# Meng-333/FastDiffSR

Hardware: AMD Instinct MI355X
Metric: 256x256 SR images/sec at T=20 (higher is better)
Workload: dtype f16x3; 1 GPU; x4 64->256, batch=16/GPU, T=20, random-init FastDiffSR UNet (inner 64, mults 1-2-4-4), 256x256, conv arithmetic f16x3 (BASELINE configs[1]); batch_per_gpu=16, global_batch=16, noise=drawn in the loop by the engine (Philox4x32-10), hipgraph=False, parallelism=dp1 (independent batches, weights broadcast once)

## Files before the change

### fastdiffsr_amd/csrc/fdsr_act_io.h

```cpp
#pragma once
#include "fdsr_kernels.h"

namespace fdsr {

typedef float f32x4 __attribute__((ext_vector_type(4)));
typedef float f32x16 __attribute__((ext_vector_type(16)));

__device__ __forceinline__ float bf16_bits_to_f32(unsigned v) { return __builtin_bit_cast(float, v << 16); }
__device__ __forceinline__ unsigned short f32_to_bf16_bits(float v) { return __builtin_bit_cast(unsigned short, (__bf16)v); }
__device__ __forceinline__ void sat_check(int* flag, f32x4 v, float lim) {
  const float m = fmaxf(fmaxf(fabsf(v.x), fabsf(v.y)), fmaxf(fabsf(v.z), fabsf(v.w)));
  if (m > lim) *flag = 1;
}
__device__ __forceinline__ int xcc_id() {
  unsigned v;
  asm volatile("s_getreg_b32 %0, hwreg(HW_REG_XCC_ID)" : "=s"(v));
  return (int)(v & (GSUM_SHARDS - 1));
}
__device__ __forceinline__ void gsum_add(unsigned long long* tab, int n, int npairs, int pair, int shard, float s1, float s2) {
  unsigned long long* g = tab + (((size_t)n * GSUM_SHARDS + shard) * npairs + pair) * 2;
  const long long a = __float2ll_rn(s1 * (float)(1 << GSUM_BITS1)), b = __float2ll_rn(s2 * (float)(1 << GSUM_BITS2));
  __hip_atomic_fetch_add(g, (unsigned long long)a, __ATOMIC_RELAXED, __HIP_MEMORY_SCOPE_WORKGROUP);
  __hip_atomic_fetch_add(g + 1, (unsigned long long)b, __ATOMIC_RELAXED, __HIP_MEMORY_SCOPE_WORKGROUP);
}
__device__ __forceinline__ float f16_bits_to_f32(unsigned v) { return (float)__builtin_bit_cast(_Float16, (unsigned short)v); }
__device__ __forceinline__ unsigned short f32_to_f16_bits(float v) {
  return __builtin_bit_cast(unsigned short, (_Float16)__builtin_amdgcn_fmed3f(v, -65504.0f, 65504.0f));
}
template <int PREC> struct ActIO;
template <> struct ActIO<PREC_F16X3> {
  typedef f32x4 Quad;
  static constexpr int ESZ = 4;
  static __device__ __forceinline__ Quad load4(const float* base, size_t idx) { return *reinterpret_cast<const f32x4*>(base + idx); }
  static __device__ __forceinline__ f32x4 widen(Quad q) { return q; }
  static __device__ __forceinline__ float load1(const float* base, size_t idx) { return base[idx]; }
  static __device__ __forceinline__ void store1(float* base, size_t idx, float v) { base[idx] = v; }
};
template <> struct ActIO<PREC_BF16> {
  typedef uint2 Quad;
  static constexpr int ESZ = 2;
  static __device__ __forceinline__ Quad load4(const float* base, size_t idx) {
    return *reinterpret_cast<const uint2*>(reinterpret_cast<const unsigned short*>(base) + idx);
  }
  static __device__ __forceinline__ f32x4 widen(Quad q) {
    f32x4 r = {__builtin_bit_cast(float, q.x << 16), __builtin_bit_cast(float, q.x & 0xffff0000u),
               __builtin_bit_cast(float, q.y << 16), __builtin_bit_cast(float, q.y & 0xffff0000u)};
    return r;
  }
  static __device__ __forceinline__ float load1(const float* base, size_t idx) {
    return bf16_bits_to_f32(reinterpret_cast<const unsigned short*>(base)[idx]);
  }
  static __device__ __forceinline__ void store1(float* base, size_t idx, float v) {
    reinterpret_cast<unsigned short*>(base)[idx] = f32_to_bf16_bits(v);
  }
};
template <> struct ActIO<PREC_F16> {
  typedef uint2 Quad;
  static constexpr int ESZ = 2;
  static __device__ __forceinline__ Quad load4(const float* base, size_t idx) {
    return *reinterpret_cast<const uint2*>(reinterpret_cast<const unsigned short*>(base) + idx);
  }
  static __device__ __forceinline__ f32x4 widen(Quad q) {
    typedef _Float16 h2 __attribute__((ext_vector_type(2)));
    const h2 a = __builtin_bit_cast(h2, q.x), b = __builtin_bit_cast(h2, q.y);
    f32x4 r = {(float)a[0], (float)a[1], (float)b[0], (float)b[1]};
    return r;
  }
  static __device__ __forceinline__ float load1(const float* base, size_t idx) {
    return f16_bits_to_f32(reinterpret_cast<const unsigned short*>(base)[idx]);
  }
  static __device__ __forceinline__ void store1(float* base, size_t idx, float v) {
    reinterpret_cast<unsigned short*>(base)[idx] = f32_to_f16_bits(v);
  }
};

template <int PREC>
__device__ __forceinline__ uint2 pack4_16(f32x4 v) {
  uint2 pk;
  if (PREC == PREC_F16) {
    pk.x = (unsigned)f32_to_f16_bits(v[0]) | ((unsigned)f32_to_f16_bits(v[1]) << 16);
    pk.y = (unsigned)f32_to_f16_bits(v[2]) | ((unsigned)f32_to_f16_bits(v[3]) << 16);
  } else {
    pk.x = (unsigned)f32_to_bf16_bits(v[0]) | ((unsigned)f32_to_bf16_bits(v[1]) << 16);
    pk.y = (unsigned)f32_to_bf16_bits(v[2]) | ((unsigned)f32_to_bf16_bits(v[3]) << 16);
  }
  return pk;
}
__device__ __forceinline__ unsigned short f32_to_16_bits(float v, int code) { return code == 2 ? f32_to_f16_bits(v) : f32_to_bf16_bits(v); }
template <int PREC>
__device__ __forceinline__ uint2 stage4_16(f32x4 v) {
  if (PREC == PREC_F16) {
    typedef _Float16 h4 __attribute__((ext_vector_type(4)));
    const h4 hb = {(_Float16)v[0], (_Float16)v[1], (_Float16)v[2], (_Float16)v[3]};
    return __builtin_bit_cast(uint2, hb);
  }
  typedef __bf16 b4_ __attribute__((ext_vector_type(4)));
  const b4_ hb = {(__bf16)v[0], (__bf16)v[1], (__bf16)v[2], (__bf16)v[3]};
  return __builtin_bit_cast(uint2, hb);
}
template <int PREC>
__device__ __forceinline__ f32x4 mfma16_k32(uint4 a, uint4 b, f32x4 c) {
  typedef __bf16 b8_ __attribute__((ext_vector_type(8)));
  typedef _Float16 h8_ __attribute__((ext_vector_type(8)));
  if (PREC == PREC_BF16) return __builtin_amdgcn_mfma_f32_16x16x32_bf16(__builtin_bit_cast(b8_, a), __builtin_bit_cast(b8_, b), c, 0, 0, 0);
  return __builtin_amdgcn_mfma_f32_16x16x32_f16(__builtin_bit_cast(h8_, a), __builtin_bit_cast(h8_, b), c, 0, 0, 0);
}
template <int PREC>
__device__ __forceinline__ f32x16 mfma32_k16(uint4 a, uint4 b, f32x16 c) {
  typedef __bf16 b8_ __attribute__((ext_vector_type(8)));
  typedef _Float16 h8_ __attribute__((ext_vector_type(8)));
  if (PREC == PREC_BF16) return __builtin_amdgcn_mfma_f32_32x32x16_bf16(__builtin_bit_cast(b8_, a), __builtin_bit_cast(b8_, b), c, 0, 0, 0);
  return __builtin_amdgcn_mfma_f32_32x32x16_f16(__builtin_bit_cast(h8_, a), __builtin_bit_cast(h8_, b), c, 0, 0, 0);
}

}
```

### fastdiffsr_amd/csrc/fdsr_conv_dev.h

```cpp
#pragma once
#include "fdsr_kernels.h"
#include "fdsr_act_io.h"

namespace fdsr {

typedef _Float16 h8 __attribute__((ext_vector_type(8)));
typedef _Float16 h4 __attribute__((ext_vector_type(4)));
typedef _Float16 h2 __attribute__((ext_vector_type(2)));
typedef __bf16 b8 __attribute__((ext_vector_type(8)));
typedef __bf16 b4 __attribute__((ext_vector_type(4)));
typedef unsigned u32x4 __attribute__((ext_vector_type(4)));

__device__ __forceinline__ float silu_fast(float v) { return v * __builtin_amdgcn_rcpf(1.0f + __expf(-v)); }

__device__ __forceinline__ int xcd_block_id(int b, int nwg) {
  const int q8 = nwg >> 3, r8 = nwg & 7, xcd = b & 7, k = b >> 3;
  return (xcd < r8 ? xcd * (q8 + 1) : r8 * (q8 + 1) + (xcd - r8) * q8) + k;
}

__device__ __forceinline__ void split2_mix(float a, float b, float lim, unsigned& hi, unsigned& lo) {
  const float ca = __builtin_amdgcn_fmed3f(a, -lim, lim), cb = __builtin_amdgcn_fmed3f(b, -lim, lim);
  const h2 h = {(_Float16)ca, (_Float16)cb};
  hi = __builtin_bit_cast(unsigned, h);
  asm("v_fma_mixlo_f16 %0, %1, -1.0, %2 op_sel:[0,0,0] op_sel_hi:[1,0,0]" : "=v"(lo) : "v"(hi), "v"(ca));
  asm("v_fma_mixhi_f16 %0, %1, -1.0, %2 op_sel:[1,0,0] op_sel_hi:[1,0,0]" : "+v"(lo) : "v"(hi), "v"(cb));
}
__device__ __forceinline__ void split4_mix(f32x4 v, float lim, uint2& hi, uint2& lo) {
#pragma unroll
  for (int e = 0; e < 4; ++e) v[e] = __builtin_amdgcn_fmed3f(v[e], -lim, lim);
  {
    const h2 h0 = {(_Float16)v[0], (_Float16)v[1]}, h1 = {(_Float16)v[2], (_Float16)v[3]};
    hi.x = __builtin_bit_cast(unsigned, h0);
    hi.y = __builtin_bit_cast(unsigned, h1);
  }
  asm("v_fma_mixlo_f16 %0, %1, -1.0, %2 op_sel:[0,0,0] op_sel_hi:[1,0,0]" : "=v"(lo.x) : "v"(hi.x), "v"(v[0]));
  asm("v_fma_mixhi_f16 %0, %1, -1.0, %2 op_sel:[1,0,0] op_sel_hi:[1,0,0]" : "+v"(lo.x) : "v"(hi.x), "v"(v[1]));
  asm("v_fma_mixlo_f16 %0, %1, -1.0, %2 op_sel:[0,0,0] op_sel_hi:[1,0,0]" : "=v"(lo.y) : "v"(hi.y), "v"(v[2]));
  asm("v_fma_mixhi_f16 %0, %1, -1.0, %2 op_sel:[1,0,0] op_sel_hi:[1,0,0]" : "+v"(lo.y) : "v"(hi.y), "v"(v[3]));
}
__device__ __forceinline__ void split4_2step(f32x4 v, float lim, h4& hi, h4& lo) {
#pragma unroll
  for (int e = 0; e < 4; ++e) v[e] = __builtin_amdgcn_fmed3f(v[e], -lim, lim);
  hi = h4{(_Float16)v.x, (_Float16)v.y, (_Float16)v.z, (_Float16)v.w};
  lo = h4{(_Float16)(v.x - (float)hi.x), (_Float16)(v.y - (float)hi.y), (_Float16)(v.z - (float)hi.z), (_Float16)(v.w - (float)hi.w)};
}

struct ChunkSrc {
  const float* base;
  int Cs, cc;
  int cbase;
  bool gn;
};
template <bool RIDER>
__device__ __forceinline__ ChunkSrc chunk_src(const ConvParams& p, int kc, int KC, int nk, int q, bool gn) {
  ChunkSrc s;
  s.cbase = kc * KC;
  s.gn = gn;
  if (RIDER && kc >= nk) {
    s.cbase -= nk * KC;
    s.gn = false;
    if (s.cbase < p.Cr0) { s.base = p.xr0; s.Cs = p.Cr0; s.cc = s.cbase + q * 4; }
    else { s.base = p.xr1; s.Cs = p.Cr1; s.cc = s.cbase - p.Cr0 + q * 4; }
  } else if (s.cbase < p.C0) { s.base = p.x0; s.Cs = p.C0; s.cc = s.cbase + q * 4; }
  else { s.base = p.x1; s.Cs = p.C1; s.cc = s.cbase - p.C0 + q * 4; }
  return s;
}

__device__ __forceinline__ f32x4 gn_act4(f32x4 v, f32x4 sc, f32x4 sh, bool plain) {
  v = v * sc + sh;
  if (!plain) { v.x = silu_fast(v.x); v.y = silu_fast(v.y); v.z = silu_fast(v.z); v.w = silu_fast(v.w); }
  return v;
}
__device__ __forceinline__ f32x4 drop4(f32x4 v, unsigned mask_bytes, float scale) {
#pragma unroll
  for (int e = 0; e < 4; ++e) v[e] *= (float)((mask_bytes >> (8 * e)) & 0xffu) * scale;
  return v;
}

template <bool RIDER>
__device__ __forceinline__ float epi_add1(const float* bias, const float* bias_r, const float* tembp, float tmul, int c) {
  float a = bias[c];
  if (RIDER) a += bias_r[c];
  a += tmul * tembp[c];
  return a;
}
template <bool RIDER>
__device__ __forceinline__ f32x4 epi_add4(const float* bias, const float* bias_r, const float* tembp, float tmul, int c) {
  f32x4 a;
#pragma unroll
  for (int r = 0; r < 4; ++r) a[r] = epi_add1<RIDER>(bias, bias_r, tembp, tmul, c + r);
  return a;
}
template <int PREC, bool OUT16>
__device__ __forceinline__ void put4(float* out, size_t idx, f32x4 v) {
  if (OUT16) *reinterpret_cast<uint2*>(reinterpret_cast<unsigned short*>(out) + idx) = pack4_16<PREC>(v);
  else *reinterpret_cast<f32x4*>(out + idx) = v;
}


}
```

### fastdiffsr_amd/csrc/fdsr_conv_h.hip

```cpp
#include "fdsr_conv_dev.h"

#include <algorithm>
#include <cstdlib>
#include <type_traits>

namespace fdsr {

template <int KS, int STRIDE, bool UP, int TH, int WN, int PREC, int KSUB>
struct ConvHCfg {
  static constexpr int TW = 32, NW = 8;
  static constexpr int KC = 16 * KSUB;
  static constexpr int NP = PREC == PREC_F16X3 ? 2 : 1;
  static constexpr int WNP = PREC == PREC_BF16 ? 1 : 2;
  static constexpr int ROWB = NP * 32 * KSUB + 16;
  static constexpr int PAD = KS / 2;
  static constexpr int HH = (TH - 1) * STRIDE + KS;
  static constexpr int HWD = (TW - 1) * STRIDE + KS;
  static constexpr int NPIX = HH * HWD;
  static constexpr int WM = NW / WN;
  static constexpr int BN = 32 * WN;
  static constexpr int MB = TH / WM;
  static constexpr int NT = 64 * NW;
  static constexpr int Q4 = 4 * KSUB;
  static constexpr int RPP = NT / Q4;
  static constexpr int NIN = (NPIX + RPP - 1) / RPP;
  static constexpr int T = KS * KS * KSUB;
  static_assert(KSUB == 1 || KS == 1, "sub-chunking is for 1x1 only");
  static constexpr int BUF_BYTES = (NPIX * ROWB + 15) / 16 * 16;
  static_assert(TH % WM == 0, "TH must be a multiple of WM");
};

#ifdef CONVH_STAMPS
__device__ unsigned long long g_h_stamps[256][2][64];
#define H_STAMP()                                                                                                  \
  do {                                                                                                             \
    if (stamp_on && si < 64) g_h_stamps[blockIdx.x][wave == 0 ? 0 : 1][si] = __builtin_amdgcn_s_memtime();         \
    ++si;                                                                                                          \
  } while (0)
#else
#define H_STAMP() do {} while (0)
#endif

template <int KS, int STRIDE, bool UP, int TH, int WN, int PREC, int KSUB, bool RIDER = false>
__global__ void __launch_bounds__(512, 2) conv_mfma_h_kernel(const ConvParams p) {
  static_assert(!RIDER || (KS == 3 && STRIDE == 1 && !UP && KSUB == 1), "the rider rides the stride-1 3x3 kernels");
  using Cfg = ConvHCfg<KS, STRIDE, UP, TH, WN, PREC, KSUB>;
  constexpr int TW = Cfg::TW, KC = Cfg::KC, NP = Cfg::NP, ROWB = Cfg::ROWB, PAD = Cfg::PAD, HWD = Cfg::HWD;
  constexpr int NPIX = Cfg::NPIX, WM = Cfg::WM, BN = Cfg::BN, MB = Cfg::MB, RPP = Cfg::RPP, NIN = Cfg::NIN, T = Cfg::T, Q4 = Cfg::Q4, NW = Cfg::NW;

  extern __shared__ __attribute__((aligned(16))) unsigned char smem_h[];
  unsigned char* sBuf0 = smem_h;
  unsigned char* sBuf1 = smem_h + Cfg::BUF_BYTES;
  const int Cin = p.C0 + p.C1;

  const int tid = threadIdx.x, lane = tid & 63, wave = tid >> 6;
  const int wn = wave % WN, wm = wave / WN;

  const int nco = p.Cout_pad / BN;
  const int tilesX = (p.Wout + TW - 1) / TW, tilesY = (p.Hout + TH - 1) / TH;
  int bid = xcd_block_id(blockIdx.x, gridDim.x);
  const int SK = p.ksplit > 1 ? p.ksplit : 1;
  const int ksi = bid % SK;
  bid /= SK;
  const int cot = bid % nco;
  int pt = bid / nco;
  const int tx = pt % tilesX;
  pt /= tilesX;
  const int ty = pt % tilesY;
  const int n = pt / tilesY;
  const int oy0 = ty * TH, ox0 = tx * TW, co0 = cot * BN;

  const bool gn = p.gn_scale != nullptr;
#ifdef CONVH_STAMPS
  int si = 0;
  const bool stamp_on = KS == 3 && STRIDE == 1 && !UP && !RIDER && PREC == CONVH_STAMP_PREC && lane == 0 && (wave == 0 || wave == 7) &&
                        blockIdx.x < 256 && Cin == CONVH_STAMP_CIN && p.Cout == CONVH_STAMP_COUT;
#endif
  H_STAMP();

  const int q = tid % Q4, row0 = tid / Q4;
  int in_pix[NIN];
#pragma unroll
  for (int i = 0; i < NIN; ++i) {
    const int pix = row0 + i * RPP;
    int v = -2;
    if (pix < NPIX) {
      const int hy = pix / HWD, hx = pix % HWD;
      const int iy = oy0 * STRIDE - PAD + hy, ix = ox0 * STRIDE - PAD + hx;
      if (UP) {
        const bool ok = iy >= 0 && iy < p.Hout && ix >= 0 && ix < p.Wout;
        v = ok ? (n * p.Hin + (iy >> 1)) * p.Win + (ix >> 1) : -1;
      } else {
        const bool ok = iy >= 0 && iy < p.Hin && ix >= 0 && ix < p.Win;
        v = ok ? (n * p.Hin + iy) * p.Win + ix : -1;
      }
    }
    in_pix[i] = v;
  }

  using IO = ActIO<PREC>;
  typedef typename IO::Quad Quad;
  Quad rin[NIN];
  Quad rin2[RIDER ? NIN : 1];
  f32x4 rsc = {1.f, 1.f, 1.f, 1.f}, rsh = {0.f, 0.f, 0.f, 0.f};
  const int nk = p.Cin_pad / KC;
  auto prefetch_to = [&](int kc, Quad* rin) {
    const ChunkSrc src = chunk_src<RIDER>(p, kc, KC, nk, q, gn);
    if (src.gn) {
      rsc = *reinterpret_cast<const f32x4*>(p.gn_scale + (size_t)n * Cin + src.cbase + q * 4);
      rsh = *reinterpret_cast<const f32x4*>(p.gn_shift + (size_t)n * Cin + src.cbase + q * 4);
    }
#pragma unroll
    for (int i = 0; i < NIN; ++i)
      rin[i] = IO::load4(src.base, (size_t)(in_pix[i] < 0 ? 0 : in_pix[i]) * src.Cs + src.cc);
  };
  auto prefetch = [&](int kc) { prefetch_to(kc, rin); };
  auto stage_from = [&](int kc, unsigned char* buf, const Quad* rin) {
    const f32x4 sc = rsc, sh = rsh;
#pragma unroll
    for (int i = 0; i < NIN; ++i) {
      if (NIN * RPP > NPIX && i == NIN - 1 && row0 + i * RPP >= NPIX) continue;
      f32x4 v = IO::widen(rin[i]);
      if (gn && !(RIDER && kc >= nk)) {
        v = gn_act4(v, sc, sh, p.gn_plain);
      } else if (PREC == PREC_F16X3 && p.sat_flag) {
        sat_check(p.sat_flag, v, 65504.f);
      }
      const float keep = in_pix[i] >= 0 ? 1.f : 0.f;
      const float lim = in_pix[i] >= 0 ? 65504.f : 0.f;
      unsigned char* dst = buf + (row0 + i * RPP) * ROWB + (q >> 2) * (NP * 32) + (q & 3) * 8;
      if (PREC == PREC_F16X3) {
        h4 hi, lo;
        split4_2step(v, lim, hi, lo);
        *reinterpret_cast<h4*>(dst) = hi;
        *reinterpret_cast<h4*>(dst + 32) = lo;
      } else {
        v = v * keep;
        *reinterpret_cast<uint2*>(dst) = stage4_16<PREC>(v);
      }
    }
  };
  auto stage = [&](int kc, unsigned char* buf) { stage_from(kc, buf, rin); };

  const uint4* wq = reinterpret_cast<const uint4*>(p.wq);
  const int nkt = RIDER ? nk + p.nkr : nk;
  uint4 Bf[T][NP];
  auto load_b_tap = [&](int kc, int tap) {
    const int ts = tap / KSUB, sub = tap % KSUB;
    const uint4* src = wq + ((((size_t)cot * (nk * KSUB) + kc * KSUB + sub) * WN + wn) * (KS * KS) + ts) * (Cfg::WNP * 64) + lane;
    if (RIDER && kc >= nk)
      src = reinterpret_cast<const uint4*>(p.wq_r) + (((size_t)cot * p.nkr + (kc - nk)) * WN + wn) * (Cfg::WNP * 64) + lane;
#pragma unroll
    for (int pl = 0; pl < NP; ++pl) Bf[tap][pl] = src[pl * 64];
  };

  const int r31 = lane & 31, h = lane >> 5;
  int abase[MB];
#pragma unroll
  for (int mb = 0; mb < MB; ++mb) {
    const int br = wm + mb * WM;
    abase[mb] = ((br * STRIDE) * HWD + r31 * STRIDE) * ROWB + 16 * h;
  }

  f32x16 acc[MB];
#pragma unroll
  for (int mb = 0; mb < MB; ++mb)
#pragma unroll
    for (int i = 0; i < 16; ++i) acc[mb][i] = 0.f;

  const int kc0 = ksi * nkt / SK, kc1 = (ksi + 1) * nkt / SK;
#pragma unroll
  for (int tap = 0; tap < T; ++tap)
    if (tap == 0 || !(RIDER && kc0 >= nk)) load_b_tap(kc0, tap);
  prefetch(kc0);
  H_STAMP();
  stage(kc0, sBuf0);
  H_STAMP();
  if (kc0 + 1 < kc1) prefetch(kc0 + 1);
  __syncthreads();
  H_STAMP();

  uint4 Af[2][MB][NP];
  const unsigned char* arow[MB];
  auto load_a = [&](int slot, int tap) {
    const int ts = tap / KSUB, sub = tap % KSUB;
    const int ky = ts / KS, kx = ts % KS;
    const int aoff = (ky * HWD + kx) * ROWB + sub * (NP * 32);
#pragma unroll
    for (int mb = 0; mb < MB; ++mb)
#pragma unroll
      for (int pl = 0; pl < NP; ++pl)
        Af[slot][mb][pl] = *reinterpret_cast<const uint4*>(arow[mb] + aoff + 32 * pl);
  };

  const int kcm = RIDER ? (kc1 < nk ? kc1 : nk) : kc1;
  for (int kc = kc0; kc < kcm; ++kc) {
    unsigned char* cur = ((kc - kc0) & 1) ? sBuf1 : sBuf0;
    unsigned char* nxt = ((kc - kc0) & 1) ? sBuf0 : sBuf1;
    const bool more = kc + 1 < kc1;
    const bool next_rider = RIDER && kc + 1 >= nk;
#pragma unroll
    for (int mb = 0; mb < MB; ++mb) arow[mb] = cur + abase[mb];
    load_a(0, 0);
#pragma unroll
    for (int tap = 0; tap < T; ++tap) {
      if (tap + 1 < T) load_a((tap + 1) & 1, tap + 1);
#pragma unroll
      for (int mb = 0; mb < MB; ++mb) {
        const uint4 ahi = Af[tap & 1][mb][0];
        if (PREC == PREC_F16X3) {
          const uint4 alo = Af[tap & 1][mb][NP - 1];
          acc[mb] = __builtin_amdgcn_mfma_f32_32x32x16_f16(__builtin_bit_cast(h8, alo), __builtin_bit_cast(h8, Bf[tap][0]), acc[mb], 0, 0, 0);
          acc[mb] = __builtin_amdgcn_mfma_f32_32x32x16_f16(__builtin_bit_cast(h8, ahi), __builtin_bit_cast(h8, Bf[tap][NP - 1]), acc[mb], 0, 0, 0);
          acc[mb] = __builtin_amdgcn_mfma_f32_32x32x16_f16(__builtin_bit_cast(h8, ahi), __builtin_bit_cast(h8, Bf[tap][0]), acc[mb], 0, 0, 0);
        } else {
          acc[mb] = mfma32_k16<PREC>(ahi, Bf[tap][0], acc[mb]);
        }
      }
      if (more && (tap == 0 || !next_rider)) load_b_tap(kc + 1, tap);
      if (tap == T / 2 && more) {
        H_STAMP();
#ifdef CONVH_KO_STAGE
        if (PREC != CONVH_KO_STAGE) {
          stage(kc + 1, nxt);
          if (kc + 2 < kc1) prefetch(kc + 2);
        }
#else
        stage(kc + 1, nxt);
        if (kc + 2 < kc1) prefetch(kc + 2);
#endif
        H_STAMP();
      }
    }
    H_STAMP();
    __syncthreads();
    H_STAMP();
  }
  if (RIDER && kc1 > nk) {
    if (kc0 < nk) {
      const float ratio = (p.w_inv_scale_dev ? *p.w_inv_scale_dev : p.w_inv_scale) / (p.w_inv_scale_r_dev ? *p.w_inv_scale_r_dev : p.w_inv_scale_r);
#pragma unroll
      for (int mb = 0; mb < MB; ++mb) acc[mb] *= ratio;
    }
    const int k0 = kc0 > nk ? kc0 : nk;
    if (k0 + 2 < kc1) prefetch_to(k0 + 2, rin2);
    auto rider_chunk = [&](int kc, Quad* r1, Quad* r2) {
      unsigned char* cur = ((kc - kc0) & 1) ? sBuf1 : sBuf0;
      unsigned char* nxt = ((kc - kc0) & 1) ? sBuf0 : sBuf1;
      (void)r2;
#pragma unroll
      for (int mb = 0; mb < MB; ++mb) arow[mb] = cur + abase[mb];
      load_a(0, T / 2);
#pragma unroll
      for (int mb = 0; mb < MB; ++mb) {
        const uint4 ahi = Af[0][mb][0];
        if (PREC == PREC_F16X3) {
          const uint4 alo = Af[0][mb][NP - 1];
          acc[mb] = __builtin_amdgcn_mfma_f32_32x32x16_f16(__builtin_bit_cast(h8, alo), __builtin_bit_cast(h8, Bf[0][0]), acc[mb], 0, 0, 0);
          acc[mb] = __builtin_amdgcn_mfma_f32_32x32x16_f16(__builtin_bit_cast(h8, ahi), __builtin_bit_cast(h8, Bf[0][NP - 1]), acc[mb], 0, 0, 0);
          acc[mb] = __builtin_amdgcn_mfma_f32_32x32x16_f16(__builtin_bit_cast(h8, ahi), __builtin_bit_cast(h8, Bf[0][0]), acc[mb], 0, 0, 0);
        } else {
          acc[mb] = mfma32_k16<PREC>(ahi, Bf[0][0], acc[mb]);
        }
      }
      if (kc + 1 < kc1) {
        load_b_tap(kc + 1, 0);
        stage_from(kc + 1, nxt, r1);
        if (kc + 3 < kc1) prefetch_to(kc + 3, r1);
      }
      __syncthreads();
    };
    for (int kc = k0; kc < kc1; kc += 2) {
      rider_chunk(kc, rin, rin2);
      if (kc + 1 < kc1) rider_chunk(kc + 1, rin2, rin);
    }
  }

  const int co = co0 + wn * 32 + r31;
  const bool cok = co < p.Cout;
  const float* tembp = p.temb ? p.temb + (size_t)n * p.temb_stride + p.temb_off : p.bias;
  const float add = epi_add1<RIDER>(p.bias, p.bias_r, tembp, p.temb ? 1.f : 0.f, cok ? co : 0);
  float s1 = 0.f, s2 = 0.f;
  const float winv_m = p.w_inv_scale_dev ? *p.w_inv_scale_dev : p.w_inv_scale;
  const float winv = RIDER ? (p.w_inv_scale_r_dev ? *p.w_inv_scale_r_dev : p.w_inv_scale_r) : winv_m;
  if (RIDER && kc1 <= nk) {
    const float ratio = winv_m / winv;
#pragma unroll
    for (int mb = 0; mb < MB; ++mb) acc[mb] *= ratio;
  }
  const bool interior = (oy0 + TH <= p.Hout) && (ox0 + TW <= p.Wout) && (co0 + BN <= p.Cout);
  if (SK > 1) {
    float* sb = p.kscratch + (size_t)ksi * p.N * p.Hout * p.Wout * p.Cout;
    if (interior) {
      float* obase = sb + ((size_t)(n * p.Hout + oy0 + wm) * p.Wout + ox0 + 4 * h) * p.Cout + co;
      const size_t rstride = (size_t)WM * p.Wout * p.Cout;
#pragma unroll
      for (int mb = 0; mb < MB; ++mb)
#pragma unroll
        for (int i = 0; i < 16; ++i) obase[mb * rstride + (size_t)((i & 3) + 8 * (i >> 2)) * p.Cout] = acc[mb][i];
    } else {
#pragma unroll
      for (int mb = 0; mb < MB; ++mb)
#pragma unroll
        for (int i = 0; i < 16; ++i) {
          const int oy = oy0 + wm + mb * WM, ox = ox0 + (i & 3) + 8 * (i >> 2) + 4 * h;
          if (cok && oy < p.Hout && ox < p.Wout) sb[((size_t)(n * p.Hout + oy) * p.Wout + ox) * p.Cout + co] = acc[mb][i];
        }
    }
    return;
  }
  auto epilogue = [&](auto out16_tag) {
    constexpr bool OUT16 = decltype(out16_tag)::value;
    auto put = [&](size_t idx, float v) {
      if (OUT16) reinterpret_cast<unsigned short*>(p.out)[idx] = PREC == PREC_F16 ? f32_to_f16_bits(v) : f32_to_bf16_bits(v);
      else p.out[idx] = v;
    };
    if (interior) {
      const size_t obase = ((size_t)(n * p.Hout + oy0 + wm) * p.Wout + ox0 + 4 * h) * p.Cout + co;
      const size_t rstride = (size_t)WM * p.Wout * p.Cout;
      float rv[MB][16];
      if (p.res) {
#pragma unroll
        for (int mb = 0; mb < MB; ++mb)
#pragma unroll
          for (int i = 0; i < 16; ++i) rv[mb][i] = IO::load1(p.res, obase + mb * rstride + (size_t)((i & 3) + 8 * (i >> 2)) * p.Cout);
      } else {
#pragma unroll
        for (int mb = 0; mb < MB; ++mb)
#pragma unroll
          for (int i = 0; i < 16; ++i) rv[mb][i] = 0.f;
      }
#pragma unroll
      for (int mb = 0; mb < MB; ++mb)
#pragma unroll
        for (int i = 0; i < 16; ++i) {
          const float v = acc[mb][i] * winv + add + rv[mb][i];
          put(obase + mb * rstride + (size_t)((i & 3) + 8 * (i >> 2)) * p.Cout, v);
          s1 += v;
          s2 += v * v;
        }
    } else {
      float rv[MB][16];
      if (p.res) {
#pragma unroll
        for (int mb = 0; mb < MB; ++mb)
#pragma unroll
          for (int i = 0; i < 16; ++i) {
            const int oy = oy0 + wm + mb * WM, ox = ox0 + (i & 3) + 8 * (i >> 2) + 4 * h;
            const bool ok = cok && oy < p.Hout && ox < p.Wout;
            rv[mb][i] = ok ? IO::load1(p.res, ((size_t)(n * p.Hout + oy) * p.Wout + ox) * p.Cout + co) : 0.f;
          }
      }
#pragma unroll
      for (int mb = 0; mb < MB; ++mb)
#pragma unroll
        for (int i = 0; i < 16; ++i) {
          const int oy = oy0 + wm + mb * WM, ox = ox0 + (i & 3) + 8 * (i >> 2) + 4 * h;
          if (cok && oy < p.Hout && ox < p.Wout) {
            float v = acc[mb][i] * winv + add;
            if (p.res) v += rv[mb][i];
            put(((size_t)(n * p.Hout + oy) * p.Wout + ox) * p.Cout + co, v);
            s1 += v;
            s2 += v * v;
          }
        }
    }
  };
  H_STAMP();
  if (prec_is16(PREC) && !p.out_f32) epilogue(std::true_type{});
  else epilogue(std::false_type{});
  H_STAMP();
  if (p.part_out) {
    float* sp = reinterpret_cast<float*>(smem_h);
    s1 += __shfl_xor(s1, 32, 64);
    s2 += __shfl_xor(s2, 32, 64);
    if (h == 0) {
      sp[(wm * BN + wn * 32 + r31) * 2 + 0] = s1;
      sp[(wm * BN + wn * 32 + r31) * 2 + 1] = s2;
    }
    __syncthreads();
    if (tid < BN && co0 + tid < p.Cout) {
      float a = 0.f, b = 0.f;
#pragma unroll
      for (int w = 0; w < WM; ++w) { a += sp[(w * BN + tid) * 2 + 0]; b += sp[(w * BN + tid) * 2 + 1]; }
      float* dst = p.part_out + (((size_t)n * (tilesX * tilesY) + ty * tilesX + tx) * p.Cout + co0 + tid) * 2;
      dst[0] = a;
      dst[1] = b;
    }
  }
  H_STAMP();
}

#ifdef CONVH_STAMPS
extern "C" int fdsr_diag_convh_stamps(unsigned long long* dst, size_t count) {
  return (int)hipMemcpyFromSymbol(dst, HIP_SYMBOL(g_h_stamps), count * sizeof(unsigned long long), 0, hipMemcpyDeviceToHost);
}
#endif

template <int NS, bool OUT16, bool CB32>
__global__ void __launch_bounds__(256) splitk_reduce_kernel(const ConvParams p, const int cb) {
  __shared__ float sred[256 * 8];
  const int tilesX = (p.Wout + 31) / 32;
  const int tile = blockIdx.x, n = blockIdx.y;
  const int tx = tile % tilesX, ty = tile / tilesX;
  const int cq = CB32 ? 8 : cb >> 2, groups = CB32 ? 32 : 256 / cq, cbase = blockIdx.z * cb;
  const int tid = threadIdx.x, c4 = tid % cq, g = tid / cq;
  const int cch = cbase + c4 * 4;
  const bool has_r = p.xr0 != nullptr, has_t = p.temb != nullptr, has_res = p.res != nullptr;
  const f32x4 bias = *reinterpret_cast<const f32x4*>(p.bias + cch);
  const f32x4 bias_r = *reinterpret_cast<const f32x4*>(has_r ? p.bias_r + cch : p.bias + cbase);
  const f32x4 temb = *reinterpret_cast<const f32x4*>(has_t ? p.temb + (size_t)n * p.temb_stride + p.temb_off + cch : p.bias + cbase);
  const float* wdev = has_r ? p.w_inv_scale_r_dev : p.w_inv_scale_dev;
  const float wload = *(wdev ? wdev : p.bias);
  const size_t slice = (size_t)p.N * p.Hout * p.Wout * p.Cout;
  const int last = p.ksplit - 1;
  const float* resp = has_res ? p.res : p.out;
  constexpr int NPX = CB32 ? 2 : 1;
  f32x4 s1 = {0.f, 0.f, 0.f, 0.f}, s2 = {0.f, 0.f, 0.f, 0.f};
  auto pixels = [&](int px0) __attribute__((always_inline)) {
    f32x4 sl[NPX][NS], rv[NPX];
    size_t o[NPX];
    bool ok[NPX];
#pragma unroll
    for (int i = 0; i < NPX; ++i) {
      const int px = px0 + i * groups;
      const int oy = ty * 2 + (px >> 5), ox = tx * 32 + (px & 31);
      ok[i] = g < groups && px < 64 && oy < p.Hout && ox < p.Wout;
      o[i] = ((size_t)(n * p.Hout + min(oy, p.Hout - 1)) * p.Wout + min(ox, p.Wout - 1)) * p.Cout + cch;
#pragma unroll
      for (int s = 0; s < NS; ++s) sl[i][s] = *reinterpret_cast<const f32x4*>(p.kscratch + (size_t)min(s, last) * slice + o[i]);
      if (OUT16) rv[i] = p.out_bf16 == 2 ? ActIO<PREC_F16>::widen(ActIO<PREC_F16>::load4(resp, o[i])) : ActIO<PREC_BF16>::widen(ActIO<PREC_BF16>::load4(resp, o[i]));
      else rv[i] = *reinterpret_cast<const f32x4*>(resp + o[i]);
    }
    __builtin_amdgcn_sched_barrier(0);
    const float winv = wdev ? wload : (has_r ? p.w_inv_scale_r : p.w_inv_scale);
    f32x4 add = bias;
#pragma unroll
    for (int e = 0; e < 4; ++e) {
      add[e] += has_r ? bias_r[e] : 0.f;
      add[e] += has_t ? temb[e] : 0.f;
    }
#pragma unroll
    for (int i = 0; i < NPX; ++i) {
      f32x4 a = sl[i][0];
#pragma unroll
      for (int s = 1; s < NS; ++s)
#pragma unroll
        for (int e = 0; e < 4; ++e) a[e] += s <= last ? sl[i][s][e] : 0.f;
      a = a * winv + add;
#pragma unroll
      for (int e = 0; e < 4; ++e) a[e] += has_res ? rv[i][e] : 0.f;
#pragma unroll
      for (int e = 0; e < 4; ++e) {
        const float v = ok[i] ? a[e] : 0.f;
        s1[e] += v;
        s2[e] += v * v;
      }
      if (ok[i]) {
        if (OUT16) {
          *reinterpret_cast<uint2*>(reinterpret_cast<unsigned short*>(p.out) + o[i]) = p.out_bf16 == 2 ? pack4_16<PREC_F16>(a) : pack4_16<PREC_BF16>(a);
        } else {
          *reinterpret_cast<f32x4*>(p.out + o[i]) = a;
        }
      }
    }
  };
  if (CB32) pixels(g);
  else for (int px0 = g; px0 < 64; px0 += groups) pixels(px0);
  if (p.part_out) {
    if (g < groups) {
      *reinterpret_cast<f32x4*>(sred + (g * cq + c4) * 8) = s1;
      *reinterpret_cast<f32x4*>(sred + (g * cq + c4) * 8 + 4) = s2;
    }
    __syncthreads();
    if (tid < cq) {
      f32x4 a = {0.f, 0.f, 0.f, 0.f}, b = a;
      for (int gg = 0; gg < groups; ++gg) {
        a += *reinterpret_cast<const f32x4*>(sred + (gg * cq + tid) * 8);
        b += *reinterpret_cast<const f32x4*>(sred + (gg * cq + tid) * 8 + 4);
      }
      float* dst = p.part_out + (((size_t)n * gridDim.x + tile) * p.Cout + cbase + tid * 4) * 2;
#pragma unroll
      for (int e = 0; e < 4; ++e) { dst[2 * e] = a[e]; dst[2 * e + 1] = b[e]; }
      if (p.gsum_out) {
        const int pair = (cbase + tid * 4) >> 1;
        const int xcd = xcc_id();
        gsum_add(p.gsum_out, n, p.Cout >> 1, pair, xcd, a[0] + a[1], b[0] + b[1]);
        gsum_add(p.gsum_out, n, p.Cout >> 1, pair + 1, xcd, a[2] + a[3], b[2] + b[3]);
      }
    }
  }
}

static hipError_t launch_splitk_reduce(const ConvParams& q, int rt, int cb, hipStream_t s) {
  const dim3 grid(rt, q.N, q.Cout / cb), block(256);
#define SKR(NS_)                                                                                                   \
  if (q.ksplit <= NS_) {                                                                                           \
    if (cb == 32) {                                                                                                \
      if (q.out_bf16) hipLaunchKernelGGL((splitk_reduce_kernel<NS_, true, true>), grid, block, 0, s, q, cb);       \
      else hipLaunchKernelGGL((splitk_reduce_kernel<NS_, false, true>), grid, block, 0, s, q, cb);                 \
    } else {                                                                                                       \
      if (q.out_bf16) hipLaunchKernelGGL((splitk_reduce_kernel<NS_, true, false>), grid, block, 0, s, q, cb);      \
      else hipLaunchKernelGGL((splitk_reduce_kernel<NS_, false, false>), grid, block, 0, s, q, cb);                \
    }                                                                                                              \
    return hipGetLastError();                                                                                      \
  }
  SKR(2) SKR(4) SKR(8) SKR(16)
#undef SKR
  return hipErrorInvalidValue;
}

template <int KS, int STRIDE, bool UP, int TH, int WN, int PREC, int KSUB, bool RIDER = false>
static hipError_t launch_h_t(const ConvParams& p, hipStream_t s, int* tiles) {
  using Cfg = ConvHCfg<KS, STRIDE, UP, TH, WN, PREC, KSUB>;
  auto kfn = conv_mfma_h_kernel<KS, STRIDE, UP, TH, WN, PREC, KSUB, RIDER>;
  const size_t lds = (size_t)2 * Cfg::BUF_BYTES;
  const int tilesX = (p.Wout + Cfg::TW - 1) / Cfg::TW, tilesY = (p.Hout + TH - 1) / TH;
  if (tiles) *tiles = tilesX * tilesY;
  const int sk = p.ksplit > 1 ? p.ksplit : 1;
  const int nwg = p.N * tilesX * tilesY * (p.Cout_pad / Cfg::BN) * sk;
  ConvParams q = p;
  q.out_bf16 = p.out_f32 ? 0 : prec_act16(PREC);
  if (KS == 3 && STRIDE == 1 && !UP && KSUB == 1 && (PREC == PREC_F16X3 || prec_is16(PREC)) && conv_k32_ok(TH, WN, PREC, q)) {
    const hipError_t e = launch_conv_k32(TH, WN, PREC, q, nwg, s);
    if (e != hipSuccess) return e;
  } else {
    if (p.gb_x0 || p.drop_mask || p.gs0) return hipErrorInvalidValue;
    hipLaunchKernelGGL(kfn, dim3(nwg), dim3(Cfg::NT), lds, s, q);
  }
  if (sk > 1 && (g_tun.knockout & 2)) {
    if (tiles) *tiles = ((p.Wout + 31) / 32) * ((p.Hout + 1) / 2);
  } else if (sk > 1) {
    const int rt = ((p.Wout + 31) / 32) * ((p.Hout + 1) / 2);
    if (tiles) *tiles = rt;
    const int cb = p.Cout % 32 == 0 ? 32 : p.Cout;
    const hipError_t e = launch_splitk_reduce(q, rt, cb, s);
    if (e != hipSuccess) return e;
  }
  return hipGetLastError();
}

template <int KS, int STRIDE, bool UP, int TH, int WN, int PREC, int KSUB, bool RIDER = false>
static hipError_t init_h_t() {
  auto kfn = conv_mfma_h_kernel<KS, STRIDE, UP, TH, WN, PREC, KSUB, RIDER>;
  return hipFuncSetAttribute(reinterpret_cast<const void*>(kfn), hipFuncAttributeMaxDynamicSharedMemorySize, 160 * 1024);
}

#define FDSR_CONVH_SHAPES(X)                                                                                   \
  X(3, 1, false, 8, 4, 1) X(3, 1, false, 4, 4, 1) X(3, 1, false, 16, 2, 1) X(3, 1, false, 8, 2, 1) X(3, 1, false, 4, 2, 1) \
  X(3, 1, false, 16, 1, 1) X(3, 1, false, 8, 1, 1) X(3, 1, false, 4, 8, 1) X(3, 1, false, 2, 8, 1)                       \
  X(3, 1, true, 4, 8, 1) X(3, 1, true, 2, 8, 1) X(3, 2, false, 4, 8, 1)                                                  \
  X(3, 1, true, 8, 4, 1) X(3, 1, true, 4, 4, 1) X(3, 1, true, 16, 2, 1) X(3, 1, true, 8, 2, 1) X(3, 1, true, 4, 2, 1)      \
  X(3, 2, false, 4, 4, 1) X(3, 2, false, 4, 2, 1)                                                                        \
  X(1, 1, false, 8, 4, 1) X(1, 1, false, 4, 4, 1) X(1, 1, false, 16, 2, 1) X(1, 1, false, 8, 2, 1) X(1, 1, false, 4, 2, 1) \
  X(1, 1, false, 16, 1, 1) X(1, 1, false, 8, 1, 1) X(1, 1, false, 4, 8, 1) X(1, 1, false, 2, 8, 1)                       \
  X(1, 1, false, 8, 4, 4) X(1, 1, false, 4, 4, 4) X(1, 1, false, 8, 2, 4) X(1, 1, false, 4, 2, 4)                         \
  X(1, 1, false, 8, 1, 4) X(1, 1, false, 4, 8, 4) X(1, 1, false, 2, 8, 4)

#define FDSR_CONVH_RIDER_SHAPES(XR) \
  XR(8, 4) XR(4, 4) XR(16, 2) XR(8, 2) XR(4, 2) XR(16, 1) XR(8, 1) XR(4, 8) XR(2, 8)

void conv_h_config(ConvKind kind, int Cout, int* TH, int* WN) {
  *WN = Cout >= 256 ? 8 : (Cout >= 128 ? 4 : (Cout >= 64 ? 2 : 1));
  if ((kind == CONV3_S2 || kind == CONV3_UP) && *WN == 1) *WN = 2;
  *TH = kind == CONV3_S2 ? 4 : 8;
}

static int pick_th(ConvKind kind, int WN, int ksub, const ConvParams& p) {
  if (kind == CONV3_S2) return 4;
  const int WM = 8 / WN;
  const int tilesX = (p.Wout + 31) / 32, nco = p.Cout_pad / (32 * WN);
  int best = -1;
  for (int th = 16; th >= 2; th >>= 1) {
    if (th % WM || th / WM > 4) continue;
    if (th < 4 && WN < 8) continue;
    if (ksub > 1 && th > 8) continue;
    const long wgs = (long)p.N * tilesX * ((p.Hout + th - 1) / th) * nco;
    best = th;
    if (wgs >= g_tun.th_min_wgs) break;
  }
  return best;
}

int conv_h_ksplit(ConvKind kind, int N, int Hout, int Wout, int Cout, int Cout_pad, int Cin_pad, int C0, int C1) {
  if (!g_tun.splitk || kind == CONV3_UP || (Cout & 3) || Cout > 1024) return 1;
  int TH, WN;
  conv_h_config(kind, Cout, &TH, &WN);
  const int ksub = (kind == CONV1 && Cin_pad % 64 == 0 && (C1 == 0 || C0 % 64 == 0)) ? 4 : 1;
  ConvParams p{};
  p.N = N; p.Hout = Hout; p.Wout = Wout; p.Cout_pad = Cout_pad;
  TH = pick_th(kind, WN, ksub, p);
  const long wgs = (long)N * ((Wout + 31) / 32) * ((Hout + TH - 1) / TH) * (Cout_pad / (32 * WN));
  const int nk = Cin_pad / (16 * ksub);
  const int target = g_tun.sk_target;
  if (wgs >= target) return 1;
  const int sk = (int)std::min<long>(std::min(16, nk / 2), (target + wgs - 1) / wgs);
  return sk >= 2 ? sk : 1;
}

bool conv_h_gnb_ok(ConvKind kind, int prec, const ConvParams& p) {
  if (kind != CONV3_S1 || prec != PREC_F16X3 || p.xr0 || p.res || p.ksplit > 1 || !p.out_f32 || p.gn_scale) return false;
  int TH, WN;
  conv_h_config(kind, p.Cout, &TH, &WN);
  if (WN == 2 && conv_k32_small_ok(kind, prec, p)) return true;
  TH = pick_th(kind, WN, 1, p);
  return conv_k32_ok(TH, WN, prec, p);
}

bool conv_h_drop_ok(ConvKind kind, int prec, const ConvParams& p) {
  if (kind != CONV3_S1 || !conv_k32_drop_ok(prec, p)) return false;
  int TH, WN;
  conv_h_config(kind, p.Cout, &TH, &WN);
  if (WN == 2 && conv_k32_small_ok(kind, prec, p)) return true;
  TH = pick_th(kind, WN, 1, p);
  return conv_k32_ok(TH, WN, prec, p);
}

bool conv_h_gnc_ok(ConvKind kind, int prec, const ConvParams& p) {
  if (!g_tun.gn_consumer || kind != CONV3_S1 || prec == PREC_F32) return false;
  int TH, WN;
  conv_h_config(kind, p.Cout, &TH, &WN);
  ConvParams q = p;
  q.gn_scale = q.gn_shift = reinterpret_cast<const float*>(p.gs_gamma);
  if ((WN == 2 || WN == 4) && conv_strip_ok(kind, prec, q)) return false;
  if (WN == 2 && conv_k32_small_ok(kind, prec, q)) return false;
  TH = pick_th(kind, WN, 1, p);
  return conv_k32_gnc_ok(TH, WN, prec, p);
}

bool conv_h_gsum_ok(ConvKind kind, int prec, const ConvParams& p, bool sub_pixel_up2) {
  if (!g_tun.gn_consumer || prec == PREC_F32 || (p.Cout & 3)) return false;
  if (p.ksplit > 1) return p.Cout % 32 == 0 && !(g_tun.knockout & 2);
  if (kind == CONV3_UP) return sub_pixel_up2 && conv_up2_k32_ok(prec, p);
  if (kind != CONV3_S1) return false;
  int TH, WN;
  conv_h_config(kind, p.Cout, &TH, &WN);
  if ((WN == 2 || WN == 4) && conv_strip_ok(kind, prec, p)) return false;
  if (WN == 2 && conv_k32_small_ok(kind, prec, p)) return true;
  TH = pick_th(kind, WN, 1, p);
  return conv_k32_ok(TH, WN, prec, p);
}

hipError_t launch_conv_h(ConvKind kind, int prec, const ConvParams& p, hipStream_t s, int* tiles) {
  int TH, WN;
  conv_h_config(kind, p.Cout, &TH, &WN);
  const int ksub = (kind == CONV1 && p.Cin_pad % 64 == 0 && (p.C1 == 0 || p.C0 % 64 == 0)) ? 4 : 1;
  if ((WN == 2 || WN == 4) && ksub == 1 && conv_strip_ok(kind, prec, p)) return launch_conv_strip(prec, p, WN, s, tiles);
  if (WN == 2 && ksub == 1 && conv_k32_small_ok(kind, prec, p)) return launch_conv_k32_small(prec, p, s, tiles);
  TH = pick_th(kind, WN, ksub, p);
  const int ks = kind == CONV1 ? 1 : 3, stride = kind == CONV3_S2 ? 2 : 1;
  const bool up = kind == CONV3_UP;
  if (p.xr0) {
    if (kind != CONV3_S1) return hipErrorInvalidValue;
#define XR(TH_, WN_)                                                                                     \
    if (TH == TH_ && WN == WN_)                                                                          \
      return prec == PREC_F16X3 ? launch_h_t<3, 1, false, TH_, WN_, PREC_F16X3, 1, true>(p, s, tiles)     \
                                : prec == PREC_F16 ? launch_h_t<3, 1, false, TH_, WN_, PREC_F16, 1, true>(p, s, tiles) : launch_h_t<3, 1, false, TH_, WN_, PREC_BF16, 1, true>(p, s, tiles);
    FDSR_CONVH_RIDER_SHAPES(XR)
#undef XR
    return hipErrorInvalidValue;
  }
#define X(KS_, ST_, UP_, TH_, WN_, KSUB_)                                                                \
  if (ks == KS_ && stride == ST_ && up == UP_ && TH == TH_ && WN == WN_ && ksub == KSUB_) {               \
    return prec == PREC_F16X3 ? launch_h_t<KS_, ST_, UP_, TH_, WN_, PREC_F16X3, KSUB_>(p, s, tiles)       \
                              : prec == PREC_F16 ? launch_h_t<KS_, ST_, UP_, TH_, WN_, PREC_F16, KSUB_>(p, s, tiles) : launch_h_t<KS_, ST_, UP_, TH_, WN_, PREC_BF16, KSUB_>(p, s, tiles);       \
  }
  FDSR_CONVH_SHAPES(X)
#undef X
  return hipErrorInvalidValue;
}

hipError_t kernels_h_init() {
  hipError_t e;
#define X(KS_, ST_, UP_, TH_, WN_, KSUB_)                                                          \
  if ((e = init_h_t<KS_, ST_, UP_, TH_, WN_, PREC_F16X3, KSUB_>()) != hipSuccess) return e;         \
  if ((e = init_h_t<KS_, ST_, UP_, TH_, WN_, PREC_BF16, KSUB_>()) != hipSuccess) return e; \
  if ((e = init_h_t<KS_, ST_, UP_, TH_, WN_, PREC_F16, KSUB_>()) != hipSuccess) return e;
  FDSR_CONVH_SHAPES(X)
#undef X
#define XR(TH_, WN_)                                                                                    \
  if ((e = init_h_t<3, 1, false, TH_, WN_, PREC_F16X3, 1, true>()) != hipSuccess) return e;              \
  if ((e = init_h_t<3, 1, false, TH_, WN_, PREC_BF16, 1, true>()) != hipSuccess) return e; \
  if ((e = init_h_t<3, 1, false, TH_, WN_, PREC_F16, 1, true>()) != hipSuccess) return e;
  FDSR_CONVH_RIDER_SHAPES(XR)
#undef XR
  if ((e = kernels_k32_init()) != hipSuccess) return e;
  return kernels_strip_init();
}

}
```

### fastdiffsr_amd/csrc/fdsr_conv_k32.hip

```cpp
#include "fdsr_conv_dev.h"

#include <type_traits>

namespace fdsr {

#ifndef XS_F16X3
#define XS_F16X3 2
#endif
#ifndef XS_BF16
#define XS_BF16 4
#endif
#ifndef K32_PIN
#define K32_PIN 1
#endif
#ifndef K32_RIDER2
#define K32_RIDER2 1
#endif
#ifndef K32_SPLIT
#define K32_SPLIT 1
#endif
#ifndef K32_SPLIT_BF16
#define K32_SPLIT_BF16 1
#endif
#ifndef K32_MIXSPLIT
#define K32_MIXSPLIT 1
#endif
#ifndef K32_PEEL
#define K32_PEEL 1
#endif
#ifndef K32_GNB_DIAG
#define K32_GNB_DIAG 0
#endif
#ifndef K32_DIAG
#define K32_DIAG 0
#endif
#ifndef K32_RFIRST
#define K32_RFIRST 1
#endif
#ifndef K32_PIN16
#define K32_PIN16 0
#endif

constexpr int K32_GNC_MAXC = 1024, K32_GNC_MAXP = K32_GNC_MAXC / 2 + 32, K32_GNC_LDS = K32_GNC_MAXP * 32 + K32_GNC_MAXC * 8;

template <int TH, int WN, int PREC, int NW_ = 8>
struct ConvK32Cfg {
  static constexpr int TW = 32, NW = NW_, KC = 32;
  static constexpr int NP = PREC == PREC_F16X3 ? 2 : 1;
  static constexpr int WNP = PREC == PREC_BF16 ? 1 : 2;
  static constexpr int ROWB = 64 * NP;
  static constexpr int HH = TH + 2, HWD = TW + 2, NPIX = HH * HWD;
  static constexpr int WM = NW / WN, BN = 32 * WN, MB = TH / WM;
  static constexpr int NT = 64 * NW;
  static constexpr int Q4 = KC / 4;
  static constexpr int RPP = NT / Q4;
  static constexpr int NIN = (NPIX + RPP - 1) / RPP;
  static constexpr int BUF_BYTES = NPIX * ROWB;
  static constexpr int LDS_BYTES = 2 * BUF_BYTES;
  static constexpr int R = 3;
  static constexpr int XS = PREC == PREC_F16X3 ? XS_F16X3 : (NW_ == 4 && TH == 8 ? 3 : XS_BF16);
  static_assert(MB == 4 || MB == 3 || MB == 2, "wave tile = 4 (small grids: 2; small workgroups in f16x3: 3) rows of 32 pixels");
  static_assert(((TH - WM + 2) * HWD + 16) * ROWB < 65536, "fragment offsets must fit the ds_read immediate");
};

template <int PREC>
__device__ __forceinline__ int k32_slot(int slot, int hx) {
  return PREC == PREC_F16X3 ? (slot ^ (hx & 7)) : (slot ^ ((hx >> 1) & 3));
}

template <int TH, int WN, int PREC, bool RIDER, int NW = 8, bool RF = (NW == 4), bool GNB = false, bool DROP = false, bool GNC = false>
__global__ void __launch_bounds__(64 * NW, 2) conv_k32_kernel(const ConvParams p) {
  using Cfg = ConvK32Cfg<TH, WN, PREC, NW>;
  constexpr int TW = Cfg::TW, KC = Cfg::KC, NP = Cfg::NP, ROWB = Cfg::ROWB, HWD = Cfg::HWD, NPIX = Cfg::NPIX;
  constexpr int WM = Cfg::WM, BN = Cfg::BN, MB = Cfg::MB, RPP = Cfg::RPP, NIN = Cfg::NIN, R = Cfg::R, XS = Cfg::XS;
  constexpr bool PIN = TH == 16 ? K32_PIN16 != 0 : K32_PIN != 0;
  constexpr bool CHAIN = PIN && !(RIDER && !RF);

  extern __shared__ __attribute__((aligned(16))) unsigned char smem_k[];
  unsigned char* sBuf0 = smem_k;
  unsigned char* sBuf1 = smem_k + Cfg::BUF_BYTES;
  const int Cin = p.C0 + p.C1;

  const int tid = threadIdx.x, lane = tid & 63, wave = tid >> 6;
  const int wn = wave % WN, wm = wave / WN;
  const int c15 = lane & 15, g = lane >> 4;

  const int nco = p.Cout_pad / BN;
  const int tilesX = (p.Wout + TW - 1) / TW, tilesY = (p.Hout + TH - 1) / TH;
  int bid = xcd_block_id(blockIdx.x, gridDim.x);
  const int SK = p.ksplit > 1 ? p.ksplit : 1;
  const int ksi = bid % SK;
  bid /= SK;
  const int cot = bid % nco;
  int pt = bid / nco;
  const int tx = pt % tilesX;
  pt /= tilesX;
  const int ty = pt % tilesY;
  const int n = pt / tilesY;
  const int oy0 = ty * TH, ox0 = tx * TW, co0 = cot * BN;

  const bool gn = GNC ? true : p.gn_scale != nullptr;

  if (NW == 4 && p.stagger > 0) {
    unsigned hwid;
    asm volatile("s_getreg_b32 %0, hwreg(HW_REG_HW_ID)" : "=s"(hwid));
    if ((hwid >> 16) & 1u) {
      const int n64 = p.stagger * (p.Cin_pad / KC + (RIDER ? p.nkr / 2 : 0));
      for (int i = 0; i < n64; i += 8) __builtin_amdgcn_s_sleep(8);
    }
  }

  const int q = tid & 7, row0 = tid >> 3;
  int in_pix[NIN];
  unsigned long long skeys = 0;
  static_assert(NIN <= 21, "swizzle keys are packed into one register pair");
#pragma unroll
  for (int i = 0; i < NIN; ++i) {
    const int pix = row0 + i * RPP;
    int v = -2;
    if (pix < NPIX) {
      const int hy = pix / HWD, hx = pix % HWD;
      const int iy = oy0 - 1 + hy, ix = ox0 - 1 + hx;
      const bool ok = iy >= 0 && iy < p.Hin && ix >= 0 && ix < p.Win;
      v = ok ? (n * p.Hin + iy) * p.Win + ix : -1;
      skeys |= (unsigned long long)k32_slot<PREC>(0, hx) << (3 * i);
    }
    in_pix[i] = v;
  }
  const int sbase = row0 * ROWB + 8 * (q & 1);

  using IO = ActIO<PREC>;
  typedef typename IO::Quad Quad;
  struct QM { Quad q; unsigned m; };
  constexpr bool RFIRST = RIDER && RF && K32_RFIRST != 0;
  constexpr bool SPLIT = K32_SPLIT != 0 && (PREC == PREC_F16X3 || K32_SPLIT_BF16 != 0) && (!RIDER || RFIRST);
  static_assert(!RFIRST || SPLIT, "the rider-first path writes whole chunks into rr1, which is sized for them only when SPLIT");
  constexpr int NA = SPLIT ? (NIN + 1) / 2 : NIN;
  typedef std::integral_constant<int, 0> I_0;
  typedef std::integral_constant<int, NA> I_A;
  typedef std::integral_constant<int, NIN> I_N;
  QM rin[NA];
  QM rr1[RIDER && SPLIT ? NIN : 1];
  QM rin2[RIDER && K32_RIDER2 && NW == 8 ? NIN : 1];
  f32x4 rsc = {1.f, 1.f, 1.f, 1.f}, rsh = {0.f, 0.f, 0.f, 0.f};
  const int nk = p.Cin_pad / KC;
  const int nk16 = p.Cin_pad / 16;
  const int nkr = RIDER ? p.nkr / 2 : 0;
  double* gnc_pr = reinterpret_cast<double*>(smem_k + Cfg::LDS_BYTES);
  float* gnc_sc = reinterpret_cast<float*>(smem_k + Cfg::LDS_BYTES + K32_GNC_MAXP * 32);
  float* gnc_sh = gnc_sc + K32_GNC_MAXC;
  int gnc_lo = 0, gnc_hi = 0, gnc_cpg = 1, gnc_q0 = 0, gnc_q1 = 0;
  constexpr int GNC_PT = (2 * K32_GNC_MAXP + Cfg::NT - 1) / Cfg::NT;
  uint4 gnc_ld[GNC ? GNC_PT : 1][GSUM_SHARDS / 2];
  constexpr int GNC_CT = (K32_GNC_MAXC + Cfg::NT - 1) / Cfg::NT;
  float gnc_gam[GNC ? GNC_CT : 1], gnc_bet[GNC ? GNC_CT : 1];
  auto gnc_issue = [&](int c_lo, int c_hi) __attribute__((always_inline)) {
    gnc_lo = c_lo; gnc_hi = c_hi;
    gnc_cpg = Cin / p.gs_G;
    gnc_q0 = (c_lo / gnc_cpg) * gnc_cpg / 2;
    gnc_q1 = ((c_hi - 1) / gnc_cpg + 1) * gnc_cpg / 2;
#pragma unroll
    for (int j = 0; j < GNC_PT; ++j) {
      const int u = tid + j * Cfg::NT, qc = min(gnc_q0 + (u >> 1), gnc_q1 - 1);
      const bool first = qc < (p.C0 >> 1);
      const unsigned long long* tab = first ? p.gs0 : p.gs1;
      const int np = (first ? p.C0 : p.C1) >> 1, ql = first ? qc : qc - (p.C0 >> 1);
#pragma unroll
      for (int sdx = 0; sdx < GSUM_SHARDS / 2; ++sdx)
        gnc_ld[j][sdx] = *reinterpret_cast<const uint4*>(tab + (((size_t)n * GSUM_SHARDS + (u & 1) * (GSUM_SHARDS / 2) + sdx) * np + ql) * 2);
    }
#pragma unroll
    for (int j = 0; j < GNC_CT; ++j) {
      const int cc = min(c_lo + tid + j * Cfg::NT, c_hi - 1);
      gnc_gam[j] = p.gs_gamma[cc];
      gnc_bet[j] = p.gs_beta[cc];
    }
  };
  auto gnc_finish = [&]() __attribute__((always_inline)) {
#pragma unroll
    for (int j = 0; j < GNC_PT; ++j) {
      const int u = tid + j * Cfg::NT, qi = gnc_q0 + (u >> 1);
      long long a = 0, b = 0;
#pragma unroll
      for (int sdx = 0; sdx < GSUM_SHARDS / 2; ++sdx) {
        a += (long long)(((unsigned long long)gnc_ld[j][sdx].y << 32) | gnc_ld[j][sdx].x);
        b += (long long)(((unsigned long long)gnc_ld[j][sdx].w << 32) | gnc_ld[j][sdx].z);
      }
      if (qi < gnc_q1) {
        gnc_pr[2 * u] = (double)a * (1.0 / (double)(1 << GSUM_BITS1));
        gnc_pr[2 * u + 1] = (double)b * (1.0 / (double)(1 << GSUM_BITS2));
      }
    }
    __syncthreads();
    const double inv = 1.0 / ((double)gnc_cpg * (double)p.Hin * (double)p.Win);
#pragma unroll
    for (int j = 0; j < GNC_CT; ++j) {
      const int c = gnc_lo + tid + j * Cfg::NT;
      if (c >= gnc_hi) break;
      const int g = c / gnc_cpg, hp = gnc_cpg >> 1;
      double s1 = 0.0, s2 = 0.0;
      for (int k = 0; k < 2 * hp; ++k) { s1 += gnc_pr[2 * (2 * (g * hp - gnc_q0) + k)]; s2 += gnc_pr[2 * (2 * (g * hp - gnc_q0) + k) + 1]; }
      const double mean = s1 * inv;
      double var = s2 * inv - mean * mean;
      var = var < 0.0 ? 0.0 : var;
      const double rstd = 1.0 / sqrt(var + (double)p.gs_eps);
      const float scv = (float)rstd * gnc_gam[j];
      gnc_sc[c - gnc_lo] = scv;
      gnc_sh[c - gnc_lo] = gnc_bet[j] - (float)mean * scv;
    }
    __syncthreads();
  };
  auto prefetch_rng = [&](int kc, QM* rin, auto i0_tag, auto i1_tag, bool load_gn) __attribute__((always_inline)) {
    constexpr int I0 = decltype(i0_tag)::value, I1 = decltype(i1_tag)::value;
    const ChunkSrc src = chunk_src<RIDER>(p, kc, KC, nk, q, gn);
    if (!GNC && src.gn && load_gn) {
      rsc = *reinterpret_cast<const f32x4*>(p.gn_scale + (size_t)n * Cin + src.cbase + q * 4);
      rsh = *reinterpret_cast<const f32x4*>(p.gn_shift + (size_t)n * Cin + src.cbase + q * 4);
    }
#pragma unroll
    for (int i = I0; i < I1; ++i) {
      const size_t pi = (size_t)(in_pix[i] < 0 ? 0 : in_pix[i]);
      rin[i - I0].q = IO::load4(src.base, pi * src.Cs + src.cc);
      if (DROP)
        rin[i - I0].m = *reinterpret_cast<const unsigned*>(p.drop_mask + ((RIDER && kc >= nk) ? (size_t)0 : pi * src.Cs + src.cc));
    }
  };
  auto prefetch_to = [&](int kc, QM* rin) __attribute__((always_inline)) { prefetch_rng(kc, rin, I_0{}, I_N{}, true); };
  auto stage_rng = [&](int kc, unsigned char* buf, const QM* rin, auto i0_tag, auto i1_tag) __attribute__((always_inline)) {
    constexpr int I0 = decltype(i0_tag)::value, I1 = decltype(i1_tag)::value;
    f32x4 sc = rsc, sh = rsh;
    if (GNC && !(RIDER && kc >= nk)) {
      sc = *reinterpret_cast<const f32x4*>(gnc_sc + (kc * KC - gnc_lo + q * 4));
      sh = *reinterpret_cast<const f32x4*>(gnc_sh + (kc * KC - gnc_lo + q * 4));
    }
#pragma unroll
    for (int i = I0; i < I1; ++i) {
      if (NIN * RPP > NPIX && i == NIN - 1 && row0 + i * RPP >= NPIX) continue;
      f32x4 v = IO::widen(rin[i - I0].q);
      if (K32_DIAG & 16) v = sc;
      if ((K32_DIAG & 1) && gn) {
        v = v + sh;
      } else if (gn && !(RIDER && kc >= nk)) {
        v = v * sc + sh;
        if (!p.gn_plain) { v.x = silu_fast(v.x); v.y = silu_fast(v.y); v.z = silu_fast(v.z); v.w = silu_fast(v.w); }
        if (DROP) {
          const unsigned m = rin[i - I0].m;
#pragma unroll
          for (int e = 0; e < 4; ++e) v[e] *= (float)((m >> (8 * e)) & 0xffu) * p.drop_scale;
        }
      } else if (PREC == PREC_F16X3 && p.sat_flag) {
        sat_check(p.sat_flag, v, 65504.f);
      }
      const int sd = sbase + i * (RPP * ROWB) + 16 * ((q >> 1) ^ (int)((skeys >> (3 * i)) & 7u));
      unsigned char* dst = buf + sd;
      if (PREC == PREC_F16X3) {
        const float lim = in_pix[i] >= 0 ? 65504.f : 0.f;
#if K32_MIXSPLIT
        uint2 hi, lo;
        split4_mix(v, lim, hi, lo);
        *reinterpret_cast<uint2*>(dst) = hi;
        *reinterpret_cast<uint2*>(buf + (sd ^ 64)) = lo;
#else
        h4 hi, lo;
        split4_2step(v, lim, hi, lo);
        *reinterpret_cast<h4*>(dst) = hi;
        *reinterpret_cast<h4*>(buf + (sd ^ 64)) = lo;
#endif
      } else {
        const float keep = in_pix[i] >= 0 ? 1.f : 0.f;
        v = v * keep;
        const uint2 hb = stage4_16<PREC>(v);
        if (K32_DIAG & 8) asm volatile("" ::"v"(hb.x), "v"(hb.y));
        else *reinterpret_cast<uint2*>(dst) = hb;
      }
    }
  };
  auto stage_from = [&](int kc, unsigned char* buf, const QM* rin) __attribute__((always_inline)) { stage_rng(kc, buf, rin, I_0{}, I_N{}); };

  const uint4* wq = reinterpret_cast<const uint4*>(p.wq);
  const int nkt = RIDER ? nk + nkr : nk;
  uint4 Wf[R][2][NP];
  const int wlane = 32 * (g & 1) + c15;
  auto load_w = [&](int kc, int tap, int slot) __attribute__((always_inline)) {
    if (K32_DIAG & 32) kc = 0;
    const uint4* src = wq + ((((size_t)cot * nk16 + 2 * kc + (g >> 1)) * WN + wn) * 9 + tap) * (Cfg::WNP * 64) + wlane;
    if (RIDER && kc >= nk)
      src = reinterpret_cast<const uint4*>(p.wq_r) + (((size_t)cot * p.nkr + 2 * (kc - nk) + (g >> 1)) * WN + wn) * (Cfg::WNP * 64) + wlane;
#pragma unroll
    for (int ch = 0; ch < 2; ++ch)
#pragma unroll
      for (int pl = 0; pl < NP; ++pl) Wf[slot][ch][pl] = src[pl * 64 + 16 * ch];
  };

  int xoff[3][NP];
#pragma unroll
  for (int kx = 0; kx < 3; ++kx) {
    const int hx = c15 + kx;
    xoff[kx][0] = (wm * HWD + hx) * ROWB + 16 * k32_slot<PREC>(g, hx);
    if (NP == 2) xoff[kx][NP - 1] = xoff[kx][0] ^ 64;
  }

  f32x4 acc[MB][2][2];
#pragma unroll
  for (int mb = 0; mb < MB; ++mb)
#pragma unroll
    for (int ph = 0; ph < 2; ++ph)
#pragma unroll
      for (int ch = 0; ch < 2; ++ch) acc[mb][ph][ch] = f32x4{0.f, 0.f, 0.f, 0.f};

  const int kc0 = ksi * nkt / SK, kc1 = (ksi + 1) * nkt / SK;
  if (RFIRST || (RIDER && kc0 >= nk)) load_w(RFIRST ? nk : kc0, 0, 0);
  else {
#pragma unroll
    for (int t = 0; t < R; ++t) load_w(kc0, t, t);
  }
  const int gm0 = RFIRST ? 0 : (kc0 < nk ? kc0 : nk), gm1 = RIDER ? (kc1 < nk ? kc1 : nk) : kc1;
  const bool gnc_on = GNC && gm1 > gm0;
  if (gnc_on) gnc_issue(gm0 * KC, gm1 * KC < Cin ? gm1 * KC : Cin);
  if (RFIRST) {
    {
      QM r0[NIN];
      prefetch_to(nk, r0);
      if (gnc_on) gnc_finish();
      stage_from(nk, sBuf0, r0);
    }
    prefetch_to(nkr > 1 ? nk + 1 : 0, rr1);
  } else if (SPLIT) {
    {
      QM r0[NIN];
      prefetch_to(kc0, r0);
      if (gnc_on) gnc_finish();
      stage_from(kc0, sBuf0, r0);
    }
    if (RIDER && kc0 >= nk && kc0 + 1 < kc1) prefetch_to(kc0 + 1, rr1);
  } else {
    prefetch_to(kc0, rin);
    if (gnc_on) gnc_finish();
    stage_from(kc0, sBuf0, rin);
    if (kc0 + 1 < kc1) prefetch_to(kc0 + 1, rin);
  }
  __syncthreads();

  uint4 Xf[XS][2][NP];
  const unsigned char* xptr[3][NP];
  auto load_x = [&](int slot, int ky, int kx, int mb) __attribute__((always_inline)) {
#pragma unroll
    for (int ph = 0; ph < 2; ++ph)
#pragma unroll
      for (int pl = 0; pl < NP; ++pl)
        Xf[slot][ph][pl] = *reinterpret_cast<const uint4*>(xptr[kx][pl] + ((mb * WM + ky) * HWD + 16 * ph) * ROWB);
  };
  auto mfma_step = [&](int xs, int ws, int mb) __attribute__((always_inline)) {
    if (PREC == PREC_F16X3) {
#pragma unroll
      for (int i = 0; i < 12; ++i) {
        const int a = CHAIN ? i / 3 : i % 4, term = CHAIN ? i % 3 : i / 4, ph = a >> 1, ch = a & 1;
        const uint4 xv = Xf[xs][ph][term == 0 ? NP - 1 : 0];
        const uint4 wv = Wf[ws][ch][term == 1 ? NP - 1 : 0];
        acc[mb][ph][ch] = __builtin_amdgcn_mfma_f32_16x16x32_f16(__builtin_bit_cast(h8, wv), __builtin_bit_cast(h8, xv),
                                                                acc[mb][ph][ch], 0, 0, 0);
        if (CHAIN && term == 2) __builtin_amdgcn_sched_barrier(0);
      }
    } else {
#pragma unroll
      for (int ph = 0; ph < 2; ++ph)
#pragma unroll
        for (int ch = 0; ch < 2; ++ch)
          acc[mb][ph][ch] = mfma16_k32<PREC>(Wf[ws][ch][0], Xf[xs][ph][0], acc[mb][ph][ch]);
    }
  };

  const int cob = co0 + wn * 32 + 4 * g;
  const bool interior = (oy0 + TH <= p.Hout) && (ox0 + TW <= p.Wout) && (co0 + BN <= p.Cout);
  const size_t obase = ((size_t)(n * p.Hout + oy0 + wm) * p.Wout + ox0 + c15) * p.Cout + cob;
  const size_t rstride = (size_t)WM * p.Wout * p.Cout, pstride = (size_t)16 * p.Cout;
  constexpr bool PEEL = K32_PEEL != 0 && (!RIDER || RFIRST);
  Quad rv[MB][2][2];
  const bool res_early = PEEL && p.res && interior && SK == 1;
  auto load_res = [&](auto q0_tag, auto q1_tag) __attribute__((always_inline)) {
    constexpr int Q0 = decltype(q0_tag)::value, Q1 = decltype(q1_tag)::value;
#pragma unroll
    for (int qi = Q0; qi < Q1; ++qi) {
      const int mb = qi >> 2, ph = (qi >> 1) & 1, ch = qi & 1;
      rv[mb][ph][ch] = IO::load4(p.res, obase + mb * rstride + ph * pstride + 16 * ch);
    }
  };
  constexpr int NQ = 4 * MB;
  typedef std::integral_constant<int, (NQ < 7 ? NQ : 7)> I_7;
  typedef std::integral_constant<int, (NQ < 11 ? NQ : 11)> I_11;
  typedef std::integral_constant<int, (NQ < 15 ? NQ : 15)> I_15;
  typedef std::integral_constant<int, NQ> I_16;

  const int kcm = RIDER ? (kc1 < nk ? kc1 : nk) : kc1;
  const int par0 = RFIRST ? nkr : 0;
  auto main_chunk = [&](int kc, auto last_tag) __attribute__((always_inline)) {
    constexpr bool LAST = decltype(last_tag)::value;
    unsigned char* cur = ((kc - kc0 + par0) & 1) ? sBuf1 : sBuf0;
    unsigned char* nxt = ((kc - kc0 + par0) & 1) ? sBuf0 : sBuf1;
    const bool more = LAST ? false : (kc + 1 < (RFIRST ? nk : kc1));
    const bool next_rider = RIDER && !RFIRST && kc + 1 >= nk;
#pragma unroll
    for (int kx = 0; kx < 3; ++kx)
#pragma unroll
      for (int pl = 0; pl < NP; ++pl) xptr[kx][pl] = cur + xoff[kx][pl];
#pragma unroll
    for (int s = 0; s < XS - 1; ++s) load_x(s, (s / MB) / 3, (s / MB) % 3, s % MB);
#pragma unroll
    for (int tap = 0; tap < 9; ++tap) {
#pragma unroll
      for (int mb = 0; mb < MB; ++mb) {
        const int s = tap * MB + mb, s2 = s + XS - 1;
        if (s2 < 9 * MB) {
          const int t2 = s2 / MB, m2 = s2 % MB;
          load_x(s2 % XS, t2 / 3, t2 % 3, m2);
        }
        if (PIN) __builtin_amdgcn_sched_barrier(0);
        mfma_step(s % XS, tap % R, mb);
        if (PIN) __builtin_amdgcn_sched_barrier(0);
      }
      if (tap + R < 9) load_w(kc, tap + R, tap % R);
      else if (more && (tap + R - 9 == 0 || !next_rider)) load_w(kc + 1, tap + R - 9, tap % R);
      if (SPLIT) {
        if (tap == 0 && more) prefetch_rng(kc + 1, rin, I_0{}, I_A{}, true);
        if (tap == 3 && more) {
          if (!(K32_DIAG & 2)) stage_rng(kc + 1, nxt, rin, I_0{}, I_A{});
          prefetch_rng(kc + 1, rin, I_A{}, I_N{}, false);
        }
        if (tap == 7 && more) {
          if (!(K32_DIAG & 2)) stage_rng(kc + 1, nxt, rin, I_A{}, I_N{});
          if (next_rider && kc + 2 < kc1) prefetch_to(kc + 2, rr1);
        }
      } else if (tap == 4 && more) {
        stage_from(kc + 1, nxt, rin);
        if (kc + 2 < kc1) prefetch_to(kc + 2, rin);
      }
      if (LAST && res_early) {
        if (tap == 0) load_res(I_0{}, I_7{});
        if (tap == 6) load_res(I_7{}, I_11{});
        if (tap == 7) load_res(I_11{}, I_15{});
        if (tap == 8) load_res(I_15{}, I_16{});
      }
    }
    __syncthreads();
  };
  if (RFIRST) {
    for (int v = 0; v < nkr; ++v) {
      unsigned char* cur = (v & 1) ? sBuf1 : sBuf0;
      unsigned char* nxt = (v & 1) ? sBuf0 : sBuf1;
#pragma unroll
      for (int pl = 0; pl < NP; ++pl) xptr[1][pl] = cur + xoff[1][pl];
#pragma unroll
      for (int mb = 0; mb < XS - 1 && mb < MB; ++mb) load_x(mb, 1, 1, mb);
#pragma unroll
      for (int mb = 0; mb < MB; ++mb) {
        if (mb + XS - 1 < MB) load_x((mb + XS - 1) % XS, 1, 1, mb + XS - 1);
        mfma_step(mb % XS, 0, mb);
      }
      if (v + 1 < nkr) {
        load_w(nk + v + 1, 0, 0);
        stage_from(nk + v + 1, nxt, rr1);
        prefetch_to(v + 2 < nkr ? nk + v + 2 : 0, rr1);
      } else {
#pragma unroll
        for (int t = 0; t < R; ++t) load_w(0, t, t);
        stage_from(0, nxt, rr1);
      }
      __syncthreads();
    }
    {
      const float ratio = (p.w_inv_scale_r_dev ? *p.w_inv_scale_r_dev : p.w_inv_scale_r) / (p.w_inv_scale_dev ? *p.w_inv_scale_dev : p.w_inv_scale);
#pragma unroll
      for (int mb = 0; mb < MB; ++mb)
#pragma unroll
        for (int ph = 0; ph < 2; ++ph)
#pragma unroll
          for (int ch = 0; ch < 2; ++ch) acc[mb][ph][ch] *= ratio;
    }
  }
  if (PEEL) {
    for (int kc = kc0; kc < kcm - 1; ++kc) main_chunk(kc, std::false_type{});
    if (kcm > kc0) main_chunk(kcm - 1, std::true_type{});
  } else {
    for (int kc = kc0; kc < kcm; ++kc) main_chunk(kc, std::false_type{});
  }
  if (RIDER && !RFIRST && kc1 > nk) {
    if (kc0 < nk) {
      const float ratio = (p.w_inv_scale_dev ? *p.w_inv_scale_dev : p.w_inv_scale) / (p.w_inv_scale_r_dev ? *p.w_inv_scale_r_dev : p.w_inv_scale_r);
#pragma unroll
      for (int mb = 0; mb < MB; ++mb)
#pragma unroll
        for (int ph = 0; ph < 2; ++ph)
#pragma unroll
          for (int ch = 0; ch < 2; ++ch) acc[mb][ph][ch] *= ratio;
    }
    const int k0 = kc0 > nk ? kc0 : nk;
    constexpr int AH = K32_RIDER2 && NW == 8 ? 2 : 1;
    if (AH == 2 && k0 + 2 < kc1) prefetch_to(k0 + 2, rin2);
    auto rider_chunk = [&](int kc, QM* r1) __attribute__((always_inline)) {
      unsigned char* cur = ((kc - kc0) & 1) ? sBuf1 : sBuf0;
      unsigned char* nxt = ((kc - kc0) & 1) ? sBuf0 : sBuf1;
#pragma unroll
      for (int pl = 0; pl < NP; ++pl) xptr[1][pl] = cur + xoff[1][pl];
#pragma unroll
      for (int mb = 0; mb < XS - 1 && mb < MB; ++mb) load_x(mb, 1, 1, mb);
#pragma unroll
      for (int mb = 0; mb < MB; ++mb) {
        if (mb + XS - 1 < MB) load_x((mb + XS - 1) % XS, 1, 1, mb + XS - 1);
        mfma_step(mb % XS, 0, mb);
      }
      if (kc + 1 < kc1) {
        load_w(kc + 1, 0, 0);
        stage_from(kc + 1, nxt, r1);
        if (kc + 1 + AH < kc1) prefetch_to(kc + 1 + AH, r1);
      }
      __syncthreads();
    };
    QM* rfirst = SPLIT ? rr1 : rin;
    if (AH == 2) {
      for (int kc = k0; kc < kc1; kc += 2) {
        rider_chunk(kc, rfirst);
        if (kc + 1 < kc1) rider_chunk(kc + 1, rin2);
      }
    } else {
      for (int kc = k0; kc < kc1; ++kc) rider_chunk(kc, rfirst);
    }
  }

  f32x4 add[2];
  bool cok[2];
  const float* tembp = p.temb ? p.temb + (size_t)n * p.temb_stride + p.temb_off : p.bias;
  const float tmul = p.temb ? 1.f : 0.f;
#pragma unroll
  for (int ch = 0; ch < 2; ++ch) {
    const int co = cob + 16 * ch;
    cok[ch] = co < p.Cout;
    add[ch] = epi_add4<RIDER>(p.bias, p.bias_r, tembp, tmul, cok[ch] ? co : 0);
  }
  const float winv_m = p.w_inv_scale_dev ? *p.w_inv_scale_dev : p.w_inv_scale;
  const float winv = RIDER && !RFIRST ? (p.w_inv_scale_r_dev ? *p.w_inv_scale_r_dev : p.w_inv_scale_r) : winv_m;
  if (RIDER && !RFIRST && kc1 <= nk) {
    const float ratio = winv_m / winv;
#pragma unroll
    for (int mb = 0; mb < MB; ++mb)
#pragma unroll
      for (int ph = 0; ph < 2; ++ph)
#pragma unroll
        for (int ch = 0; ch < 2; ++ch) acc[mb][ph][ch] *= ratio;
  }
  if (SK > 1) {
    float* sb = p.kscratch + (size_t)ksi * p.N * p.Hout * p.Wout * p.Cout;
#pragma unroll
    for (int mb = 0; mb < MB; ++mb)
#pragma unroll
      for (int ph = 0; ph < 2; ++ph)
#pragma unroll
        for (int ch = 0; ch < 2; ++ch) {
          const int oy = oy0 + wm + mb * WM, ox = ox0 + 16 * ph + c15;
          if (interior || (cok[ch] && oy < p.Hout && ox < p.Wout))
            *reinterpret_cast<f32x4*>(sb + obase + mb * rstride + ph * pstride + 16 * ch) = acc[mb][ph][ch];
        }
    return;
  }
  f32x4 s1[2], s2[2];
#pragma unroll
  for (int ch = 0; ch < 2; ++ch) s1[ch] = s2[ch] = f32x4{0.f, 0.f, 0.f, 0.f};
  auto epilogue = [&](auto out16_tag) __attribute__((always_inline)) {
    constexpr bool OUT16 = decltype(out16_tag)::value;
    if (interior) {
      if (p.res && !res_early) {
#pragma unroll
        for (int mb = 0; mb < MB; ++mb)
#pragma unroll
          for (int ph = 0; ph < 2; ++ph)
#pragma unroll
            for (int ch = 0; ch < 2; ++ch) rv[mb][ph][ch] = IO::load4(p.res, obase + mb * rstride + ph * pstride + 16 * ch);
      }
#pragma unroll
      for (int mb = 0; mb < MB; ++mb)
#pragma unroll
        for (int ph = 0; ph < 2; ++ph)
#pragma unroll
          for (int ch = 0; ch < 2; ++ch) {
            f32x4 v = acc[mb][ph][ch] * winv + add[ch];
            if (p.res) v += IO::widen(rv[mb][ph][ch]);
            put4<PREC, OUT16>(p.out, obase + mb * rstride + ph * pstride + 16 * ch, v);
            if (!(K32_DIAG & 4)) {
              s1[ch] += v;
              s2[ch] += v * v;
            }
          }
    } else {
#pragma unroll
      for (int mb = 0; mb < MB; ++mb)
#pragma unroll
        for (int ph = 0; ph < 2; ++ph)
#pragma unroll
          for (int ch = 0; ch < 2; ++ch) {
            const int oy = oy0 + wm + mb * WM, ox = ox0 + 16 * ph + c15;
            if (cok[ch] && oy < p.Hout && ox < p.Wout) {
              const size_t idx = obase + mb * rstride + ph * pstride + 16 * ch;
              f32x4 v = acc[mb][ph][ch] * winv + add[ch];
              if (p.res) v += IO::widen(IO::load4(p.res, idx));
              put4<PREC, OUT16>(p.out, idx, v);
              s1[ch] += v;
              s2[ch] += v * v;
            }
          }
    }
  };
  auto epilogue_gnb = [&](auto int_tag) __attribute__((always_inline)) {
    constexpr bool INTERIOR = decltype(int_tag)::value;
    const int Ct = p.Cout, cpg = Ct / p.gb_G;
    const bool hm = p.gb_mask != nullptr;
    const unsigned char* mk = hm ? p.gb_mask : reinterpret_cast<const unsigned char*>(p.gb_scale);
    const float ds = p.gb_drop;
#pragma unroll
    for (int ch = 0; ch < 2; ++ch) {
      const int cs = cok[ch] ? cob + 16 * ch : 0;
      const f32x4 gsc = *reinterpret_cast<const f32x4*>(p.gb_scale + (size_t)n * Ct + cs);
      const f32x4 gsh = *reinterpret_cast<const f32x4*>(p.gb_shift + (size_t)n * Ct + cs);
      f32x4 gme, grs;
#pragma unroll
      for (int r = 0; r < 4; ++r) {
        const int grp = (cs + r) / cpg;
        gme[r] = p.gb_stats[((size_t)n * p.gb_G + grp) * 2];
        grs[r] = p.gb_stats[((size_t)n * p.gb_G + grp) * 2 + 1];
      }
      const float* xb;
      int xcs;
      if (cs < p.gb_C0) { xb = p.gb_x0 + cs; xcs = p.gb_C0; }
      else { xb = p.gb_x1 + (cs - p.gb_C0); xcs = Ct - p.gb_C0; }
      f32x4 xq[MB][2];
      unsigned mq[MB][2];
#pragma unroll
      for (int mb = 0; mb < MB; ++mb) {
        const int oy = min(oy0 + wm + mb * WM, p.Hout - 1);
#pragma unroll
        for (int ph = 0; ph < 2; ++ph) {
          const size_t pix = (size_t)(n * p.Hout + oy) * p.Wout + min(ox0 + 16 * ph + c15, p.Wout - 1);
          if (K32_GNB_DIAG & 2) { xq[mb][ph] = gsc; mq[mb][ph] = 0x01010101u; continue; }
          xq[mb][ph] = *reinterpret_cast<const f32x4*>(xb + pix * xcs);
          mq[mb][ph] = *reinterpret_cast<const unsigned*>(mk + (hm ? pix * Ct + cs : (size_t)0));
        }
      }
#pragma unroll
      for (int mb = 0; mb < MB; ++mb) {
        const int oy = oy0 + wm + mb * WM;
#pragma unroll
        for (int ph = 0; ph < 2; ++ph) {
          const int ox = ox0 + 16 * ph + c15;
          const bool ok = INTERIOR || (cok[ch] && oy < p.Hout && ox < p.Wout);
          const f32x4 v = acc[mb][ph][ch] * winv + add[ch];
          const f32x4 x = xq[mb][ph];
          const unsigned m = mq[mb][ph];
          f32x4 gq, gx;
#pragma unroll
          for (int r = 0; r < 4; ++r) {
            float d = v[r];
            if (hm) d = ((m >> (8 * r)) & 0xffu) ? d * ds : 0.f;
            const float xh = (x[r] - gme[r]) * grs[r];
            float gg = d;
            if (!p.gb_plain && !(K32_GNB_DIAG & 1)) {
              const float u = fmaf(x[r], gsc[r], gsh[r]);
              const float sg = __builtin_amdgcn_rcpf(1.0f + __expf(-u));
              gg = d * (sg * (1.0f + u * (1.0f - sg)));
            }
            gq[r] = gg;
            gx[r] = gg * xh;
          }
          if (ok) {
            *reinterpret_cast<f32x4*>(p.out + obase + mb * rstride + ph * pstride + 16 * ch) = gq;
            s1[ch] += gq;
            s2[ch] += gx;
          }
        }
      }
    }
  };
  if constexpr (GNB) {
    if (interior) epilogue_gnb(std::true_type{});
    else epilogue_gnb(std::false_type{});
  } else {
    if (prec_is16(PREC) && !p.out_f32) epilogue(std::true_type{});
    else epilogue(std::false_type{});
  }
  if (p.part_out) {
    float vals[16];
#pragma unroll
    for (int ch = 0; ch < 2; ++ch)
#pragma unroll
      for (int r = 0; r < 4; ++r) { vals[ch * 8 + r * 2] = s1[ch][r]; vals[ch * 8 + r * 2 + 1] = s2[ch][r]; }
#pragma unroll
    for (int half = 8; half >= 1; half >>= 1) {
      const bool up = (c15 & half) != 0;
#pragma unroll
      for (int i = 0; i < half; ++i) {
        const float keep = up ? vals[i + half] : vals[i];
        const float send = up ? vals[i] : vals[i + half];
        vals[i] = keep + __shfl_xor(send, half, 64);
      }
    }
    float* sp = reinterpret_cast<float*>(smem_k);
    {
      const int ch = c15 >> 3, r = (c15 >> 1) & 3, st = c15 & 1;
      sp[(wm * BN + wn * 32 + 16 * ch + 4 * g + r) * 2 + st] = vals[0];
    }
    __syncthreads();
    float a_keep = 0.f, b_keep = 0.f;
    if (tid < BN && co0 + tid < p.Cout) {
      float a = 0.f, b = 0.f;
#pragma unroll
      for (int w = 0; w < WM; ++w) { a += sp[(w * BN + tid) * 2 + 0]; b += sp[(w * BN + tid) * 2 + 1]; }
      a_keep = a; b_keep = b;
      float* dst = p.part_out + (((size_t)n * (tilesX * tilesY) + ty * tilesX + tx) * p.Cout + co0 + tid) * 2;
      dst[0] = a;
      dst[1] = b;
    }
    if (p.gsum_out) {
      const float a2 = a_keep + __shfl_xor(a_keep, 1, 64), b2 = b_keep + __shfl_xor(b_keep, 1, 64);
      if (tid < BN && !(tid & 1) && co0 + tid < p.Cout) gsum_add(p.gsum_out, n, p.Cout >> 1, (co0 + tid) >> 1, xcc_id(), a2, b2);
    }
  }
}

template <int TH, int WN, int PREC>
struct ConvUp2K32Cfg {
  static constexpr int TW = 32, KC = 32;
  static constexpr int NP = PREC == PREC_F16X3 ? 2 : 1;
  static constexpr int WNP = PREC == PREC_BF16 ? 1 : 2;
  static constexpr int ROWB = 64 * NP;
  static constexpr int HH = TH + 1, HWD = TW + 2, NPIX = HH * HWD;
  static constexpr int WM = 8 / WN, BN = 32 * WN, MB = TH / WM;
  static constexpr int RPP = 512 / 8, NIN = (NPIX + RPP - 1) / RPP;
  static constexpr int BUF_BYTES = NPIX * ROWB;
  static constexpr int R = 4;
  static_assert(MB == 2, "two source rows per wave");
};

template <int TH, int WN, int PREC>
__global__ void __launch_bounds__(512, 2) conv_up2_k32_kernel(const ConvParams p) {
  using Cfg = ConvUp2K32Cfg<TH, WN, PREC>;
  constexpr int TW = Cfg::TW, KC = Cfg::KC, NP = Cfg::NP, ROWB = Cfg::ROWB, HWD = Cfg::HWD, NPIX = Cfg::NPIX;
  constexpr int WM = Cfg::WM, BN = Cfg::BN, MB = Cfg::MB, RPP = Cfg::RPP, NIN = Cfg::NIN, R = Cfg::R;

  extern __shared__ __attribute__((aligned(16))) unsigned char smem_uk[];
  unsigned char* sBuf0 = smem_uk;
  unsigned char* sBuf1 = smem_uk + Cfg::BUF_BYTES;

  const int tid = threadIdx.x, lane = tid & 63, wave = tid >> 6;
  const int wn = wave % WN, wm = wave / WN;
  const int c15 = lane & 15, g = lane >> 4;

  const int nco = p.Cout_pad / BN;
  const int tilesX = (p.Win + TW - 1) / TW, tilesY = (p.Hin + TH - 1) / TH;
  const int bid = xcd_block_id(blockIdx.x, gridDim.x);
  const int cot = bid % nco;
  int pt = bid / nco;
  const int py = pt & 1;
  pt >>= 1;
  const int tx = pt % tilesX;
  pt /= tilesX;
  const int ty = pt % tilesY;
  const int n = pt / tilesY;
  const int oy0 = ty * TH, ox0 = tx * TW, co0 = cot * BN;

  const int q = tid & 7, row0 = tid >> 3;
  int in_pix[NIN];
  unsigned skeys = 0;
#pragma unroll
  for (int i = 0; i < NIN; ++i) {
    const int pix = row0 + i * RPP;
    int v = -2;
    if (pix < NPIX) {
      const int hy = pix / HWD, hx = pix % HWD;
      const int iy = oy0 - 1 + py + hy, ix = ox0 - 1 + hx;
      const bool ok = iy >= 0 && iy < p.Hin && ix >= 0 && ix < p.Win;
      v = ok ? (n * p.Hin + iy) * p.Win + ix : -1;
      skeys |= (unsigned)k32_slot<PREC>(0, hx) << (3 * i);
    }
    in_pix[i] = v;
  }
  const int sbase = row0 * ROWB + 8 * (q & 1);
  using IO = ActIO<PREC>;
  typedef typename IO::Quad Quad;
  Quad rin[NIN];
  auto prefetch = [&](int kc) {
    const size_t coff = (size_t)kc * KC + q * 4;
#pragma unroll
    for (int i = 0; i < NIN; ++i) rin[i] = IO::load4(p.x0, (size_t)(in_pix[i] < 0 ? 0 : in_pix[i]) * p.C0 + coff);
  };
  auto stage = [&](unsigned char* buf) {
#pragma unroll
    for (int i = 0; i < NIN; ++i) {
      if (NIN * RPP > NPIX && i == NIN - 1 && row0 + i * RPP >= NPIX) continue;
      f32x4 v = IO::widen(rin[i]);
      const int sd = sbase + i * (RPP * ROWB) + 16 * ((q >> 1) ^ (int)((skeys >> (3 * i)) & 7u));
      if (PREC == PREC_F16X3) {
        if (p.sat_flag) sat_check(p.sat_flag, v, 65504.f);
        const float lim = in_pix[i] >= 0 ? 65504.f : 0.f;
#pragma unroll
        for (int e = 0; e < 4; ++e) v[e] = __builtin_amdgcn_fmed3f(v[e], -lim, lim);
        uint2 hi, lo;
        {
          const h2 h0 = {(_Float16)v[0], (_Float16)v[1]}, h1 = {(_Float16)v[2], (_Float16)v[3]};
          hi.x = __builtin_bit_cast(unsigned, h0);
          hi.y = __builtin_bit_cast(unsigned, h1);
        }
        asm("v_fma_mixlo_f16 %0, %1, -1.0, %2 op_sel:[0,0,0] op_sel_hi:[1,0,0]" : "=v"(lo.x) : "v"(hi.x), "v"(v[0]));
        asm("v_fma_mixhi_f16 %0, %1, -1.0, %2 op_sel:[1,0,0] op_sel_hi:[1,0,0]" : "+v"(lo.x) : "v"(hi.x), "v"(v[1]));
        asm("v_fma_mixlo_f16 %0, %1, -1.0, %2 op_sel:[0,0,0] op_sel_hi:[1,0,0]" : "=v"(lo.y) : "v"(hi.y), "v"(v[2]));
        asm("v_fma_mixhi_f16 %0, %1, -1.0, %2 op_sel:[1,0,0] op_sel_hi:[1,0,0]" : "+v"(lo.y) : "v"(hi.y), "v"(v[3]));
        *reinterpret_cast<uint2*>(buf + sd) = hi;
        *reinterpret_cast<uint2*>(buf + (sd ^ 64)) = lo;
      } else {
        const float keep = in_pix[i] >= 0 ? 1.f : 0.f;
        v = v * keep;
        *reinterpret_cast<uint2*>(buf + sd) = stage4_16<PREC>(v);
      }
    }
  };

  const uint4* wq = reinterpret_cast<const uint4*>(p.wq);
  const int nk = p.Cin_pad / KC, nk16 = p.Cin_pad / 16;
  uint4 Wf[R][2][NP];
  const int wlane = 32 * (g & 1) + c15;
  auto load_w = [&](int kc, int slot) {
    const uint4* src = wq + ((((((size_t)cot * nk16 + 2 * kc + (g >> 1)) * WN + wn) * 2 + py) * 8 + slot) * (Cfg::WNP * 64)) + wlane;
#pragma unroll
    for (int ch = 0; ch < 2; ++ch)
#pragma unroll
      for (int pl = 0; pl < NP; ++pl) Wf[slot % R][ch][pl] = src[pl * 64 + 16 * ch];
  };

  int xoff[3][NP];
#pragma unroll
  for (int c = 0; c < 3; ++c) {
    const int hx = c15 + c;
    xoff[c][0] = (wm * HWD + hx) * ROWB + 16 * k32_slot<PREC>(g, hx);
    if (NP == 2) xoff[c][NP - 1] = xoff[c][0] ^ 64;
  }

  f32x4 acc[MB][2][2][2];
#pragma unroll
  for (int mb = 0; mb < MB; ++mb)
#pragma unroll
    for (int px = 0; px < 2; ++px)
#pragma unroll
      for (int ph = 0; ph < 2; ++ph)
#pragma unroll
        for (int ch = 0; ch < 2; ++ch) acc[mb][px][ph][ch] = f32x4{0.f, 0.f, 0.f, 0.f};

#pragma unroll
  for (int sl = 0; sl < R; ++sl) load_w(0, sl);
  prefetch(0);
  stage(sBuf0);
  if (nk > 1) prefetch(1);
  __syncthreads();

  uint4 Xf[2][2][NP];
  const unsigned char* xptr[3][NP];
  auto load_x = [&](int xs, int slot, int mb) {
    const int a = (slot >> 1) & 1, c = (slot >> 2) + (slot & 1);
#pragma unroll
    for (int ph = 0; ph < 2; ++ph)
#pragma unroll
      for (int pl = 0; pl < NP; ++pl)
        Xf[xs][ph][pl] = *reinterpret_cast<const uint4*>(xptr[c][pl] + ((mb * WM + a) * HWD + 16 * ph) * ROWB);
  };
  auto mfma_step = [&](int xs, int slot, int mb) {
    const int px = slot >> 2, ws = slot % R;
    if (PREC == PREC_F16X3) {
#pragma unroll
      for (int ph = 0; ph < 2; ++ph)
#pragma unroll
        for (int ch = 0; ch < 2; ++ch) {
#pragma unroll
          for (int term = 0; term < 3; ++term) {
            const uint4 xv = Xf[xs][ph][term == 0 ? NP - 1 : 0];
            const uint4 wv = Wf[ws][ch][term == 1 ? NP - 1 : 0];
            acc[mb][px][ph][ch] = __builtin_amdgcn_mfma_f32_16x16x32_f16(__builtin_bit_cast(h8, wv), __builtin_bit_cast(h8, xv),
                                                                        acc[mb][px][ph][ch], 0, 0, 0);
          }
          __builtin_amdgcn_sched_barrier(0);
        }
    } else {
#pragma unroll
      for (int ph = 0; ph < 2; ++ph)
#pragma unroll
        for (int ch = 0; ch < 2; ++ch)
          acc[mb][px][ph][ch] = mfma16_k32<PREC>(Wf[ws][ch][0], Xf[xs][ph][0], acc[mb][px][ph][ch]);
    }
  };

  for (int kc = 0; kc < nk; ++kc) {
    unsigned char* cur = (kc & 1) ? sBuf1 : sBuf0;
    unsigned char* nxt = (kc & 1) ? sBuf0 : sBuf1;
    const bool more = kc + 1 < nk;
#pragma unroll
    for (int c = 0; c < 3; ++c)
#pragma unroll
      for (int pl = 0; pl < NP; ++pl) xptr[c][pl] = cur + xoff[c][pl];
    load_x(0, 0, 0);
#pragma unroll
    for (int slot = 0; slot < 8; ++slot) {
#pragma unroll
      for (int mb = 0; mb < MB; ++mb) {
        const int s = slot * MB + mb;
        if (s + 1 < 8 * MB) load_x((s + 1) & 1, (s + 1) / MB, (s + 1) % MB);
        __builtin_amdgcn_sched_barrier(0);
        mfma_step(s & 1, slot, mb);
        __builtin_amdgcn_sched_barrier(0);
      }
      if (slot + R < 8) load_w(kc, slot + R);
      else if (more) load_w(kc + 1, slot + R - 8);
      if (slot == 3 && more) {
        stage(nxt);
        if (kc + 2 < nk) prefetch(kc + 2);
      }
    }
    __syncthreads();
  }

  const int cob = co0 + wn * 32 + 4 * g;
  const float winv = p.w_inv_scale_dev ? *p.w_inv_scale_dev : p.w_inv_scale;
  f32x4 add[2];
  bool cok[2];
  const float* tembp = p.temb ? p.temb + (size_t)n * p.temb_stride + p.temb_off : p.bias;
  const float tmul = p.temb ? 1.f : 0.f;
#pragma unroll
  for (int ch = 0; ch < 2; ++ch) {
    const int co = cob + 16 * ch;
    cok[ch] = co < p.Cout;
    add[ch] = epi_add4<false>(p.bias, p.bias_r, tembp, tmul, cok[ch] ? co : 0);
  }
  f32x4 s1[2], s2[2];
#pragma unroll
  for (int ch = 0; ch < 2; ++ch) s1[ch] = s2[ch] = f32x4{0.f, 0.f, 0.f, 0.f};
  constexpr bool OUT16 = prec_is16(PREC);
#pragma unroll
  for (int mb = 0; mb < MB; ++mb)
#pragma unroll
    for (int px = 0; px < 2; ++px)
#pragma unroll
      for (int ph = 0; ph < 2; ++ph)
#pragma unroll
        for (int ch = 0; ch < 2; ++ch) {
          const int sy = oy0 + wm + mb * WM, sx = ox0 + 16 * ph + c15;
          if (cok[ch] && sy < p.Hin && sx < p.Win) {
            const size_t idx = ((size_t)(n * p.Hout + 2 * sy + py) * p.Wout + 2 * sx + px) * p.Cout + cob + 16 * ch;
            const f32x4 v = acc[mb][px][ph][ch] * winv + add[ch];
            put4<PREC, OUT16>(p.out, idx, v);
            s1[ch] += v;
            s2[ch] += v * v;
          }
        }
  if (p.part_out) {
    float vals[16];
#pragma unroll
    for (int ch = 0; ch < 2; ++ch)
#pragma unroll
      for (int r = 0; r < 4; ++r) { vals[ch * 8 + r * 2] = s1[ch][r]; vals[ch * 8 + r * 2 + 1] = s2[ch][r]; }
#pragma unroll
    for (int half = 8; half >= 1; half >>= 1) {
      const bool up = (c15 & half) != 0;
#pragma unroll
      for (int i = 0; i < half; ++i) {
        const float keep = up ? vals[i + half] : vals[i];
        const float send = up ? vals[i] : vals[i + half];
        vals[i] = keep + __shfl_xor(send, half, 64);
      }
    }
    float* sp = reinterpret_cast<float*>(smem_uk);
    {
      const int ch = c15 >> 3, r = (c15 >> 1) & 3, st = c15 & 1;
      sp[(wm * BN + wn * 32 + 16 * ch + 4 * g + r) * 2 + st] = vals[0];
    }
    __syncthreads();
    float a_keep = 0.f, b_keep = 0.f;
    if (tid < BN && co0 + tid < p.Cout) {
      float a = 0.f, b = 0.f;
#pragma unroll
      for (int w = 0; w < WM; ++w) { a += sp[(w * BN + tid) * 2 + 0]; b += sp[(w * BN + tid) * 2 + 1]; }
      a_keep = a; b_keep = b;
      float* dst = p.part_out + (((size_t)n * (tilesX * tilesY * 2) + (ty * tilesX + tx) * 2 + py) * p.Cout + co0 + tid) * 2;
      dst[0] = a;
      dst[1] = b;
    }
    if (p.gsum_out) {
      const float a2 = a_keep + __shfl_xor(a_keep, 1, 64), b2 = b_keep + __shfl_xor(b_keep, 1, 64);
      if (tid < BN && !(tid & 1) && co0 + tid < p.Cout) gsum_add(p.gsum_out, n, p.Cout >> 1, (co0 + tid) >> 1, xcc_id(), a2, b2);
    }
  }
}

bool conv_up2_k32_ok(int prec, const ConvParams& p) {
  if (!(g_tun.k32 & FDSR_K32_UP2) || !(g_tun.k32 & (prec_is16(prec) ? FDSR_K32_BF16 : FDSR_K32_F16X3))) return false;
  return p.C1 == 0 && p.C0 % 32 == 0 && p.C0 == p.Cin_pad && p.Cout % 4 == 0 && !p.gn_scale && !p.res;
}

template <int TH, int WN, int PREC>
static hipError_t launch_up2_k32_t(const ConvParams& q, int nwg, hipStream_t s) {
  using Cfg = ConvUp2K32Cfg<TH, WN, PREC>;
  hipLaunchKernelGGL((conv_up2_k32_kernel<TH, WN, PREC>), dim3(nwg), dim3(512), (size_t)2 * Cfg::BUF_BYTES, s, q);
  return hipGetLastError();
}

#define FDSR_UP2_K32_SHAPES(X) X(8, 2) X(4, 4) X(2, 8)

hipError_t launch_conv_up2_k32(int TH, int WN, int prec, const ConvParams& q, int nwg, hipStream_t s) {
#define X(TH_, WN_)                                                                                    \
  if (TH == TH_ && WN == WN_)                                                                          \
    return prec == PREC_F16X3 ? launch_up2_k32_t<TH_, WN_, PREC_F16X3>(q, nwg, s) : prec == PREC_F16 ? launch_up2_k32_t<TH_, WN_, PREC_F16>(q, nwg, s) : launch_up2_k32_t<TH_, WN_, PREC_BF16>(q, nwg, s);
  FDSR_UP2_K32_SHAPES(X)
#undef X
  return hipErrorInvalidValue;
}

#define FDSR_K32_SHAPES(X) X(16, 2) X(8, 4) X(4, 8) X(8, 2) X(4, 4) X(2, 8)

bool conv_k32_ok(int TH, int WN, int prec, const ConvParams& p) {
  if (!(g_tun.k32 & (prec_is16(prec) ? FDSR_K32_BF16 : FDSR_K32_F16X3))) return false;
  if (TH == 16 && p.xr0 && !(g_tun.k32 & FDSR_K32_RIDER_16ROW)) return false;
  if (TH * WN != 32 && !(TH * WN == 16 && (g_tun.k32 & FDSR_K32_SMALL_GRID_2ROW))) return false;
  if (WN != 2 && WN != 4 && WN != 8) return false;
  if (p.Cin_pad % 32 || (p.C0 + p.C1) != p.Cin_pad) return false;
  if (p.C1 != 0 && p.C0 % 32) return false;
  if (p.Cout % 4) return false;
  if (p.xr0) {
    if (p.nkr % 2 || (p.Cr0 + p.Cr1) != p.nkr * 16) return false;
    if (p.Cr1 != 0 && p.Cr0 % 32) return false;
  }
  return true;
}

template <int TH, int WN, int PREC, bool RIDER, int NW = 8, bool RF = (NW == 4), bool GNB = false, bool DROP = false, bool GNC = false>
static hipError_t launch_k32_t(const ConvParams& q, int nwg, hipStream_t s) {
  using Cfg = ConvK32Cfg<TH, WN, PREC, NW>;
  hipLaunchKernelGGL((conv_k32_kernel<TH, WN, PREC, RIDER, NW, RF, GNB, DROP, GNC>), dim3(nwg), dim3(Cfg::NT), (size_t)Cfg::LDS_BYTES + (GNC ? K32_GNC_LDS : 0), s, q);
  return hipGetLastError();
}

bool conv_k32_drop_ok(int prec, const ConvParams& q) {
  if (prec != PREC_F16X3 || !q.drop_mask || !q.gn_scale || q.gn_plain || q.C1 != 0 || q.ksplit > 1 || q.gb_x0) return false;
  return !q.xr0 || (g_tun.k32 & FDSR_K32_RIDER_FIRST_8WAVE);
}

static bool k32_gnb_ok(int prec, const ConvParams& q) {
  if (prec != PREC_F16X3 || !q.out_f32 || q.xr0 || q.res || q.ksplit > 1 || !q.gb_scale || !q.gb_shift || !q.gb_stats) return false;
  if (q.gb_G <= 0 || q.Cout % q.gb_G || q.Cout % 4) return false;
  return q.gb_x1 ? (q.gb_C0 % 4 == 0 && q.gb_C0 > 0 && q.gb_C0 < q.Cout) : q.gb_C0 == q.Cout;
}

static int k32_small_rows(int prec, bool rider) { return prec_is16(prec) && !rider ? 8 : 6; }

bool conv_k32_small_ok(ConvKind kind, int prec, const ConvParams& p) {
  if (!(g_tun.k32 & FDSR_K32_SMALL_WG_F16X3) || kind != CONV3_S1 || p.ksplit > 1 || p.Cout_pad != 64) return false;
  if (prec_is16(prec) && !(g_tun.k32 & FDSR_K32_SMALL_WG_BF16)) return false;
  if (p.xr0 && !(g_tun.k32 & (prec_is16(prec) ? FDSR_K32_SMALL_WG_RIDER_BF16 : FDSR_K32_SMALL_WG_RIDER_F16X3))) return false;
  if (!conv_k32_ok(8, 4, prec, p)) return false;
  const int th = k32_small_rows(prec, p.xr0 != nullptr);
  const long wgs = (long)p.N * ((p.Wout + 31) / 32) * ((p.Hout + th - 1) / th);
  return wgs >= g_tun.k32_sb_min_wgs;
}

hipError_t launch_conv_k32_small(int prec, const ConvParams& p, hipStream_t s, int* tiles) {
  const int th = k32_small_rows(prec, p.xr0 != nullptr);
  const int tilesX = (p.Wout + 31) / 32, tilesY = (p.Hout + th - 1) / th;
  if (tiles) *tiles = tilesX * tilesY;
  const int nwg = p.N * tilesX * tilesY;
  ConvParams q = p;
  q.out_bf16 = p.out_f32 ? 0 : prec_act16(prec);
  q.stagger = g_tun.k32_stagger;
  if (q.gb_x0) return k32_gnb_ok(prec, q) ? launch_k32_t<6, 2, PREC_F16X3, false, 4, true, true>(q, nwg, s) : hipErrorInvalidValue;
  if (q.drop_mask) {
    if (!conv_k32_drop_ok(prec, q)) return hipErrorInvalidValue;
    return q.xr0 ? launch_k32_t<6, 2, PREC_F16X3, true, 4, true, false, true>(q, nwg, s) : launch_k32_t<6, 2, PREC_F16X3, false, 4, true, false, true>(q, nwg, s);
  }
  if (prec == PREC_F16X3)
    return q.xr0 ? launch_k32_t<6, 2, PREC_F16X3, true, 4>(q, nwg, s) : launch_k32_t<6, 2, PREC_F16X3, false, 4>(q, nwg, s);
  if (prec == PREC_F16) return q.xr0 ? launch_k32_t<6, 2, PREC_F16, true, 4>(q, nwg, s) : launch_k32_t<8, 2, PREC_F16, false, 4>(q, nwg, s);
  return q.xr0 ? launch_k32_t<6, 2, PREC_BF16, true, 4>(q, nwg, s) : launch_k32_t<8, 2, PREC_BF16, false, 4>(q, nwg, s);
}

#define FDSR_K32_GNC_SHAPES(X) X(8, 2) X(4, 4) X(2, 8)
bool conv_k32_gnc_ok(int TH, int WN, int prec, const ConvParams& p) {
  if (TH * WN != 16 || !conv_k32_ok(TH, WN, prec, p)) return false;
  if (p.gb_x0 || p.drop_mask || p.gn_plain || (p.C0 & 1) || (p.C1 & 1)) return false;
  const int Cin = p.C0 + p.C1;
  return Cin <= K32_GNC_MAXC && p.gs_G > 0 && Cin % p.gs_G == 0 && ((Cin / p.gs_G) & 1) == 0;
}

hipError_t launch_conv_k32(int TH, int WN, int prec, const ConvParams& q, int nwg, hipStream_t s) {
  if (q.gs0) {
    if (!conv_k32_gnc_ok(TH, WN, prec, q)) return hipErrorInvalidValue;
    const bool rf = q.xr0 && q.ksplit <= 1 && (g_tun.k32 & FDSR_K32_RIDER_FIRST_8WAVE);
#define X(TH_, WN_)                                                                                                      \
    if (TH == TH_ && WN == WN_) {                                                                                        \
      if (rf) return prec == PREC_F16X3 ? launch_k32_t<TH_, WN_, PREC_F16X3, true, 8, true, false, false, true>(q, nwg, s)   \
                                        : prec == PREC_F16 ? launch_k32_t<TH_, WN_, PREC_F16, true, 8, true, false, false, true>(q, nwg, s) : launch_k32_t<TH_, WN_, PREC_BF16, true, 8, true, false, false, true>(q, nwg, s);    \
      if (q.xr0) return prec == PREC_F16X3 ? launch_k32_t<TH_, WN_, PREC_F16X3, true, 8, false, false, false, true>(q, nwg, s)  \
                                           : prec == PREC_F16 ? launch_k32_t<TH_, WN_, PREC_F16, true, 8, false, false, false, true>(q, nwg, s) : launch_k32_t<TH_, WN_, PREC_BF16, true, 8, false, false, false, true>(q, nwg, s);   \
      return prec == PREC_F16X3 ? launch_k32_t<TH_, WN_, PREC_F16X3, false, 8, false, false, false, true>(q, nwg, s)      \
                                : prec == PREC_F16 ? launch_k32_t<TH_, WN_, PREC_F16, false, 8, false, false, false, true>(q, nwg, s) : launch_k32_t<TH_, WN_, PREC_BF16, false, 8, false, false, false, true>(q, nwg, s);       \
    }
    FDSR_K32_GNC_SHAPES(X)
#undef X
    return hipErrorInvalidValue;
  }
#define X(TH_, WN_)                                                                                             \
  if (TH == TH_ && WN == WN_) {                                                                                 \
    if (q.gb_x0) return k32_gnb_ok(prec, q) ? launch_k32_t<TH_, WN_, PREC_F16X3, false, 8, false, true>(q, nwg, s) : hipErrorInvalidValue; \
    if (q.drop_mask) {                                                                                          \
      if (!conv_k32_drop_ok(prec, q)) return hipErrorInvalidValue;                                              \
      return q.xr0 ? launch_k32_t<TH_, WN_, PREC_F16X3, true, 8, true, false, true>(q, nwg, s)                  \
                   : launch_k32_t<TH_, WN_, PREC_F16X3, false, 8, false, false, true>(q, nwg, s);               \
    }                                                                                                           \
    if (q.xr0 && q.ksplit <= 1 && (g_tun.k32 & FDSR_K32_RIDER_FIRST_8WAVE))                                                           \
      return prec == PREC_F16X3 ? launch_k32_t<TH_, WN_, PREC_F16X3, true, 8, true>(q, nwg, s)                  \
                                : prec == PREC_F16 ? launch_k32_t<TH_, WN_, PREC_F16, true, 8, true>(q, nwg, s) : launch_k32_t<TH_, WN_, PREC_BF16, true, 8, true>(q, nwg, s);                  \
    if (q.xr0) return prec == PREC_F16X3 ? launch_k32_t<TH_, WN_, PREC_F16X3, true>(q, nwg, s)                  \
                                         : prec == PREC_F16 ? launch_k32_t<TH_, WN_, PREC_F16, true>(q, nwg, s) : launch_k32_t<TH_, WN_, PREC_BF16, true>(q, nwg, s);                  \
    return prec == PREC_F16X3 ? launch_k32_t<TH_, WN_, PREC_F16X3, false>(q, nwg, s)                            \
                              : prec == PREC_F16 ? launch_k32_t<TH_, WN_, PREC_F16, false>(q, nwg, s) : launch_k32_t<TH_, WN_, PREC_BF16, false>(q, nwg, s);                            \
  }
  FDSR_K32_SHAPES(X)
#undef X
  return hipErrorInvalidValue;
}

template <int TH, int WN, int PREC, bool RIDER, int NW = 8, bool RF = (NW == 4), bool GNB = false, bool DROP = false, bool GNC = false>
static hipError_t init_k32_t() {
  auto kfn = conv_k32_kernel<TH, WN, PREC, RIDER, NW, RF, GNB, DROP, GNC>;
  return hipFuncSetAttribute(reinterpret_cast<const void*>(kfn), hipFuncAttributeMaxDynamicSharedMemorySize, 160 * 1024);
}

template <int TH, int WN, int PREC>
static hipError_t init_up2_k32_t() {
  auto kfn = conv_up2_k32_kernel<TH, WN, PREC>;
  return hipFuncSetAttribute(reinterpret_cast<const void*>(kfn), hipFuncAttributeMaxDynamicSharedMemorySize, 160 * 1024);
}

hipError_t kernels_k32_init() {
  hipError_t e;
#define X(TH_, WN_)                                                                 \
  if ((e = init_up2_k32_t<TH_, WN_, PREC_F16X3>()) != hipSuccess) return e;         \
  if ((e = init_up2_k32_t<TH_, WN_, PREC_BF16>()) != hipSuccess) return e; \
  if ((e = init_up2_k32_t<TH_, WN_, PREC_F16>()) != hipSuccess) return e;
  FDSR_UP2_K32_SHAPES(X)
#undef X
#define X(TH_, WN_)                                                                        \
  if ((e = init_k32_t<TH_, WN_, PREC_F16X3, false>()) != hipSuccess) return e;             \
  if ((e = init_k32_t<TH_, WN_, PREC_F16X3, true>()) != hipSuccess) return e;              \
  if ((e = init_k32_t<TH_, WN_, PREC_BF16, false>()) != hipSuccess) return e;              \
  if ((e = init_k32_t<TH_, WN_, PREC_F16, false>()) != hipSuccess) return e;              \
  if ((e = init_k32_t<TH_, WN_, PREC_BF16, true>()) != hipSuccess) return e;                \
  if ((e = init_k32_t<TH_, WN_, PREC_F16, true>()) != hipSuccess) return e;                \
  if ((e = init_k32_t<TH_, WN_, PREC_F16X3, true, 8, true>()) != hipSuccess) return e;     \
  if ((e = init_k32_t<TH_, WN_, PREC_F16X3, false, 8, false, true>()) != hipSuccess) return e; \
  if ((e = init_k32_t<TH_, WN_, PREC_F16X3, false, 8, false, false, true>()) != hipSuccess) return e; \
  if ((e = init_k32_t<TH_, WN_, PREC_F16X3, true, 8, true, false, true>()) != hipSuccess) return e; \
  if ((e = init_k32_t<TH_, WN_, PREC_BF16, true, 8, true>()) != hipSuccess) return e; \
  if ((e = init_k32_t<TH_, WN_, PREC_F16, true, 8, true>()) != hipSuccess) return e;
  FDSR_K32_SHAPES(X)
#undef X
#define X(TH_, WN_)                                                                                                     \
  if ((e = init_k32_t<TH_, WN_, PREC_F16X3, false, 8, false, false, false, true>()) != hipSuccess) return e;            \
  if ((e = init_k32_t<TH_, WN_, PREC_F16X3, true, 8, false, false, false, true>()) != hipSuccess) return e;             \
  if ((e = init_k32_t<TH_, WN_, PREC_F16X3, true, 8, true, false, false, true>()) != hipSuccess) return e;              \
  if ((e = init_k32_t<TH_, WN_, PREC_BF16, false, 8, false, false, false, true>()) != hipSuccess) return e;             \
  if ((e = init_k32_t<TH_, WN_, PREC_F16, false, 8, false, false, false, true>()) != hipSuccess) return e;             \
  if ((e = init_k32_t<TH_, WN_, PREC_BF16, true, 8, false, false, false, true>()) != hipSuccess) return e;              \
  if ((e = init_k32_t<TH_, WN_, PREC_F16, true, 8, false, false, false, true>()) != hipSuccess) return e;              \
  if ((e = init_k32_t<TH_, WN_, PREC_BF16, true, 8, true, false, false, true>()) != hipSuccess) return e; \
  if ((e = init_k32_t<TH_, WN_, PREC_F16, true, 8, true, false, false, true>()) != hipSuccess) return e;
  FDSR_K32_GNC_SHAPES(X)
#undef X
  if ((e = init_k32_t<6, 2, PREC_F16X3, false, 4>()) != hipSuccess) return e;
  if ((e = init_k32_t<6, 2, PREC_F16X3, true, 4>()) != hipSuccess) return e;
  if ((e = init_k32_t<6, 2, PREC_F16X3, false, 4, true, true>()) != hipSuccess) return e;
  if ((e = init_k32_t<6, 2, PREC_F16X3, false, 4, true, false, true>()) != hipSuccess) return e;
  if ((e = init_k32_t<6, 2, PREC_F16X3, true, 4, true, false, true>()) != hipSuccess) return e;
  if ((e = init_k32_t<6, 2, PREC_BF16, true, 4>()) != hipSuccess) return e;
  if ((e = init_k32_t<6, 2, PREC_F16, true, 4>()) != hipSuccess) return e;
  return hipSuccess;
}

}
```

### fastdiffsr_amd/csrc/fdsr_conv_up2.hip

```cpp
#include "fdsr_conv_dev.h"

namespace fdsr {

template <int TH, int WN, int PREC>
struct ConvUp2Cfg {
  static constexpr int TW = 32, KC = 16;
  static constexpr int NP = PREC == PREC_F16X3 ? 2 : 1;
  static constexpr int WNP = PREC == PREC_BF16 ? 1 : 2;
  static constexpr int ROWB = NP * 32 + 16;
  static constexpr int HH = TH + 1, HWD = TW + 2, NPIX = HH * HWD;
  static constexpr int WM = 8 / WN, BN = 32 * WN, MB = TH / WM;
  static constexpr int RPP = 512 / 4, NIN = (NPIX + RPP - 1) / RPP;
  static constexpr int BUF_BYTES = (NPIX * ROWB + 15) / 16 * 16;
  static_assert(TH % WM == 0 && MB <= 2, "at most 2 source rows x 2 column parities per wave");
};

template <int TH, int WN, int PREC>
__global__ void __launch_bounds__(512, 2) conv_up2_h_kernel(const ConvParams p) {
  using Cfg = ConvUp2Cfg<TH, WN, PREC>;
  constexpr int TW = Cfg::TW, KC = Cfg::KC, NP = Cfg::NP, ROWB = Cfg::ROWB, HWD = Cfg::HWD, NPIX = Cfg::NPIX;
  constexpr int WM = Cfg::WM, BN = Cfg::BN, MB = Cfg::MB, RPP = Cfg::RPP, NIN = Cfg::NIN;

  extern __shared__ __attribute__((aligned(16))) unsigned char smem_u[];
  unsigned char* sBuf0 = smem_u;
  unsigned char* sBuf1 = smem_u + Cfg::BUF_BYTES;

  const int tid = threadIdx.x, lane = tid & 63, wave = tid >> 6;
  const int wn = wave % WN, wm = wave / WN;
  const int r31 = lane & 31, h = lane >> 5;

  const int nco = p.Cout_pad / BN;
  const int tilesX = (p.Win + TW - 1) / TW, tilesY = (p.Hin + TH - 1) / TH;
  const int bid = xcd_block_id(blockIdx.x, gridDim.x);
  const int cot = bid % nco;
  int pt = bid / nco;
  const int py = pt & 1;
  pt >>= 1;
  const int tx = pt % tilesX;
  pt /= tilesX;
  const int ty = pt % tilesY;
  const int n = pt / tilesY;
  const int oy0 = ty * TH, ox0 = tx * TW, co0 = cot * BN;

  const int q = tid & 3, row0 = tid >> 2;
  int in_pix[NIN];
#pragma unroll
  for (int i = 0; i < NIN; ++i) {
    const int pix = row0 + i * RPP;
    const int hy = pix / HWD, hx = pix % HWD;
    const int iy = oy0 - 1 + py + hy, ix = ox0 - 1 + hx;
    const bool ok = pix < NPIX && iy >= 0 && iy < p.Hin && ix >= 0 && ix < p.Win;
    in_pix[i] = ok ? (n * p.Hin + iy) * p.Win + ix : -1;
  }
  using IO = ActIO<PREC>;
  typename IO::Quad rin[NIN];
  auto prefetch = [&](int kc) {
    const size_t coff = (size_t)kc * KC + q * 4;
#pragma unroll
    for (int i = 0; i < NIN; ++i)
      rin[i] = IO::load4(p.x0, (size_t)(in_pix[i] < 0 ? 0 : in_pix[i]) * p.C0 + coff);
  };
  auto stage = [&](unsigned char* buf) {
#pragma unroll
    for (int i = 0; i < NIN; ++i) {
      if (NIN * RPP > NPIX && i == NIN - 1 && row0 + i * RPP >= NPIX) continue;
      f32x4 v = IO::widen(rin[i]);
      const float keep = in_pix[i] >= 0 ? 1.f : 0.f;
      const float lim = in_pix[i] >= 0 ? 65504.f : 0.f;
      unsigned char* dst = buf + (row0 + i * RPP) * ROWB + q * 8;
      if (PREC == PREC_F16X3) {
        if (p.sat_flag) sat_check(p.sat_flag, v, 65504.f);
        h4 hi, lo;
        split4_2step(v, lim, hi, lo);
        *reinterpret_cast<h4*>(dst) = hi;
        *reinterpret_cast<h4*>(dst + 32) = lo;
      } else {
        v = v * keep;
        *reinterpret_cast<uint2*>(dst) = stage4_16<PREC>(v);
      }
    }
  };

  const uint4* wq = reinterpret_cast<const uint4*>(p.wq);
  const int nk = p.Cin_pad / KC;
  uint4 Bf[8][NP];
  auto load_b_slot = [&](int kc, int slot) {
    const uint4* src = wq + (((((size_t)cot * nk + kc) * WN + wn) * 2 + py) * 8 + slot) * (Cfg::WNP * 64) + lane;
#pragma unroll
    for (int pl = 0; pl < NP; ++pl) Bf[slot][pl] = src[pl * 64];
  };

  int abase[MB];
#pragma unroll
  for (int mb = 0; mb < MB; ++mb) abase[mb] = ((wm + mb * WM) * HWD + r31) * ROWB + 16 * h;

  f32x16 acc[MB][2];
#pragma unroll
  for (int mb = 0; mb < MB; ++mb)
#pragma unroll
    for (int px = 0; px < 2; ++px)
#pragma unroll
      for (int i = 0; i < 16; ++i) acc[mb][px][i] = 0.f;

#pragma unroll
  for (int sl = 0; sl < 8; ++sl) load_b_slot(0, sl);
  prefetch(0);
  stage(sBuf0);
  if (nk > 1) prefetch(1);
  __syncthreads();

  auto mma = [&](f32x16& c, const uint4 (&a)[NP], const uint4 (&b)[NP]) {
    if (PREC == PREC_F16X3) {
      c = __builtin_amdgcn_mfma_f32_32x32x16_f16(__builtin_bit_cast(h8, a[NP - 1]), __builtin_bit_cast(h8, b[0]), c, 0, 0, 0);
      c = __builtin_amdgcn_mfma_f32_32x32x16_f16(__builtin_bit_cast(h8, a[0]), __builtin_bit_cast(h8, b[NP - 1]), c, 0, 0, 0);
      c = __builtin_amdgcn_mfma_f32_32x32x16_f16(__builtin_bit_cast(h8, a[0]), __builtin_bit_cast(h8, b[0]), c, 0, 0, 0);
    } else {
      c = mfma32_k16<PREC>(a[0], b[0], c);
    }
  };

  for (int kc = 0; kc < nk; ++kc) {
    unsigned char* cur = (kc & 1) ? sBuf1 : sBuf0;
    unsigned char* nxt = (kc & 1) ? sBuf0 : sBuf1;
    const bool more = kc + 1 < nk;
#pragma unroll
    for (int mb = 0; mb < MB; ++mb) {
      uint4 Af[2][3][NP];
#pragma unroll
      for (int a = 0; a < 2; ++a)
#pragma unroll
        for (int c = 0; c < 3; ++c)
#pragma unroll
          for (int pl = 0; pl < NP; ++pl)
            Af[a][c][pl] = *reinterpret_cast<const uint4*>(cur + abase[mb] + (a * HWD + c) * ROWB + 32 * pl);
#pragma unroll
      for (int slot = 0; slot < 8; ++slot) {
        const int px = slot >> 2, a = (slot >> 1) & 1, b = slot & 1;
        mma(acc[mb][px], Af[a][px + b], Bf[slot]);
        if (mb == MB - 1 && more) load_b_slot(kc + 1, slot);
        if (mb == MB - 1 && slot == 1 && more) {
          stage(nxt);
          if (kc + 2 < nk) prefetch(kc + 2);
        }
      }
    }
    __syncthreads();
  }

  const int co = co0 + wn * 32 + r31;
  const bool cok = co < p.Cout;
  const float winv = p.w_inv_scale_dev ? *p.w_inv_scale_dev : p.w_inv_scale;
  const float* tembp = p.temb ? p.temb + (size_t)n * p.temb_stride + p.temb_off : p.bias;
  const float add = epi_add1<false>(p.bias, p.bias_r, tembp, p.temb ? 1.f : 0.f, cok ? co : 0);
  float s1 = 0.f, s2 = 0.f;
  const bool interior = (oy0 + TH <= p.Hin) && (ox0 + TW <= p.Win) && (co0 + BN <= p.Cout);
  if (interior) {
#pragma unroll
    for (int mb = 0; mb < MB; ++mb) {
      const int Y = 2 * (oy0 + wm + mb * WM) + py;
      const size_t rowp = ((size_t)(n * p.Hout + Y) * p.Wout + 2 * (ox0 + 4 * h)) * p.Cout + co;
#pragma unroll
      for (int px = 0; px < 2; ++px)
#pragma unroll
        for (int i = 0; i < 16; ++i) {
          const float v = acc[mb][px][i] * winv + add;
          IO::store1(p.out, rowp + (size_t)(2 * ((i & 3) + 8 * (i >> 2)) + px) * p.Cout, v);
          s1 += v;
          s2 += v * v;
        }
    }
  } else {
#pragma unroll
    for (int mb = 0; mb < MB; ++mb)
#pragma unroll
      for (int px = 0; px < 2; ++px)
#pragma unroll
        for (int i = 0; i < 16; ++i) {
          const int sy = oy0 + wm + mb * WM, sx = ox0 + (i & 3) + 8 * (i >> 2) + 4 * h;
          if (cok && sy < p.Hin && sx < p.Win) {
            const float v = acc[mb][px][i] * winv + add;
            IO::store1(p.out, ((size_t)(n * p.Hout + 2 * sy + py) * p.Wout + 2 * sx + px) * p.Cout + co, v);
            s1 += v;
            s2 += v * v;
          }
        }
  }
  if (p.part_out) {
    float* sp = reinterpret_cast<float*>(smem_u);
    s1 += __shfl_xor(s1, 32, 64);
    s2 += __shfl_xor(s2, 32, 64);
    if (h == 0) {
      sp[(wm * BN + wn * 32 + r31) * 2 + 0] = s1;
      sp[(wm * BN + wn * 32 + r31) * 2 + 1] = s2;
    }
    __syncthreads();
    if (tid < BN && co0 + tid < p.Cout) {
      float a = 0.f, b = 0.f;
#pragma unroll
      for (int w = 0; w < WM; ++w) { a += sp[(w * BN + tid) * 2 + 0]; b += sp[(w * BN + tid) * 2 + 1]; }
      float* dst = p.part_out + (((size_t)n * (tilesX * tilesY * 2) + (ty * tilesX + tx) * 2 + py) * p.Cout + co0 + tid) * 2;
      dst[0] = a;
      dst[1] = b;
    }
  }
}

template <int TH, int WN, int PREC>
static hipError_t launch_up2_t(const ConvParams& p, hipStream_t s, int* tiles) {
  using Cfg = ConvUp2Cfg<TH, WN, PREC>;
  auto kfn = conv_up2_h_kernel<TH, WN, PREC>;
  const int tilesX = (p.Win + Cfg::TW - 1) / Cfg::TW, tilesY = (p.Hin + TH - 1) / TH;
  if (tiles) *tiles = tilesX * tilesY * 2;
  const int nwg = p.N * tilesX * tilesY * 2 * (p.Cout_pad / Cfg::BN);
  if (conv_up2_k32_ok(PREC, p)) return launch_conv_up2_k32(TH, WN, PREC, p, nwg, s);
  hipLaunchKernelGGL(kfn, dim3(nwg), dim3(512), (size_t)2 * Cfg::BUF_BYTES, s, p);
  return hipGetLastError();
}

hipError_t launch_conv_up2_h(int prec, const ConvParams& p, hipStream_t s, int* tiles) {
  int TH, WN;
  conv_h_config(CONV3_UP, p.Cout, &TH, &WN);
#define X(TH_, WN_)                                                                           \
  if (WN == WN_) return prec == PREC_F16X3 ? launch_up2_t<TH_, WN_, PREC_F16X3>(p, s, tiles)  \
                                           : prec == PREC_F16 ? launch_up2_t<TH_, WN_, PREC_F16>(p, s, tiles) : launch_up2_t<TH_, WN_, PREC_BF16>(p, s, tiles);
  X(8, 2) X(4, 4) X(2, 8)
#undef X
  return hipErrorInvalidValue;
}

}
```

Measured before the change: 74.68 images/s.

## Fold saturation checks per thread and specialize k32 conv for GN+SiLU and chunk kind

The per-element saturation check, which could issue a global store inside the staging loop, becomes a running per-thread max that is tested once after the K loop, removing a branch and store from the hot path. The k32 conv kernel also gains a compile-time GS variant, selected when GroupNorm with SiLU is active, so the gn and gn_plain runtime checks are resolved at compile time. Chunk-kind tags let rider and main chunks resolve their source selection statically, and the rider-first loop is restructured with its last iteration peeled. The cost is more kernel instantiations, longer compile time and more code size.

```diff
diff --git a/fastdiffsr_amd/csrc/fdsr_act_io.h b/fastdiffsr_amd/csrc/fdsr_act_io.h
--- a/fastdiffsr_amd/csrc/fdsr_act_io.h
+++ b/fastdiffsr_amd/csrc/fdsr_act_io.h
@@ -11,6 +11,12 @@
 __device__ __forceinline__ void sat_check(int* flag, f32x4 v, float lim) {
   const float m = fmaxf(fmaxf(fabsf(v.x), fabsf(v.y)), fmaxf(fabsf(v.z), fabsf(v.w)));
   if (m > lim) *flag = 1;
+}
+__device__ __forceinline__ float sat_fold(float m, f32x4 v) {
+  return fmaxf(m, fmaxf(fmaxf(fabsf(v.x), fabsf(v.y)), fmaxf(fabsf(v.z), fabsf(v.w))));
+}
+__device__ __forceinline__ void sat_raise(int* flag, float m, float lim) {
+  if (flag && m > lim) *flag = 1;
 }
 __device__ __forceinline__ int xcc_id() {
   unsigned v;
diff --git a/fastdiffsr_amd/csrc/fdsr_conv_dev.h b/fastdiffsr_amd/csrc/fdsr_conv_dev.h
--- a/fastdiffsr_amd/csrc/fdsr_conv_dev.h
+++ b/fastdiffsr_amd/csrc/fdsr_conv_dev.h
@@ -51,12 +51,16 @@
   int cbase;
   bool gn;
 };
-template <bool RIDER>
+enum ChunkKind { CHUNK_MAIN = 0, CHUNK_RIDER = 1, CHUNK_ANY = 2 };
+template <int KIND>
+__device__ __forceinline__ bool chunk_is_rider(int kc, int nk) { return KIND == CHUNK_ANY ? kc >= nk : KIND == CHUNK_RIDER; }
+
+template <bool RIDER, int KIND = (RIDER ? CHUNK_ANY : CHUNK_MAIN)>
 __device__ __forceinline__ ChunkSrc chunk_src(const ConvParams& p, int kc, int KC, int nk, int q, bool gn) {
   ChunkSrc s;
   s.cbase = kc * KC;
   s.gn = gn;
-  if (RIDER && kc >= nk) {
+  if (RIDER && chunk_is_rider<KIND>(kc, nk)) {
     s.cbase -= nk * KC;
     s.gn = false;
     if (s.cbase < p.Cr0) { s.base = p.xr0; s.Cs = p.Cr0; s.cc = s.cbase + q * 4; }
diff --git a/fastdiffsr_amd/csrc/fdsr_conv_h.hip b/fastdiffsr_amd/csrc/fdsr_conv_h.hip
--- a/fastdiffsr_amd/csrc/fdsr_conv_h.hip
+++ b/fastdiffsr_amd/csrc/fdsr_conv_h.hip
@@ -103,6 +103,7 @@
   Quad rin[NIN];
   Quad rin2[RIDER ? NIN : 1];
   f32x4 rsc = {1.f, 1.f, 1.f, 1.f}, rsh = {0.f, 0.f, 0.f, 0.f};
+  float satm = 0.f;
   const int nk = p.Cin_pad / KC;
   auto prefetch_to = [&](int kc, Quad* rin) {
     const ChunkSrc src = chunk_src<RIDER>(p, kc, KC, nk, q, gn);
@@ -123,8 +124,8 @@
       f32x4 v = IO::widen(rin[i]);
       if (gn && !(RIDER && kc >= nk)) {
         v = gn_act4(v, sc, sh, p.gn_plain);
-      } else if (PREC == PREC_F16X3 && p.sat_flag) {
-        sat_check(p.sat_flag, v, 65504.f);
+      } else if (PREC == PREC_F16X3) {
+        satm = sat_fold(satm, v);
       }
       const float keep = in_pix[i] >= 0 ? 1.f : 0.f;
       const float lim = in_pix[i] >= 0 ? 65504.f : 0.f;
@@ -275,6 +276,7 @@
       if (kc + 1 < kc1) rider_chunk(kc + 1, rin2, rin);
     }
   }
+  if (PREC == PREC_F16X3) sat_raise(p.sat_flag, satm, 65504.f);
 
   const int co = co0 + wn * 32 + r31;
   const bool cok = co < p.Cout;
diff --git a/fastdiffsr_amd/csrc/fdsr_conv_k32.hip b/fastdiffsr_amd/csrc/fdsr_conv_k32.hip
--- a/fastdiffsr_amd/csrc/fdsr_conv_k32.hip
+++ b/fastdiffsr_amd/csrc/fdsr_conv_k32.hip
@@ -68,7 +68,7 @@
   return PREC == PREC_F16X3 ? (slot ^ (hx & 7)) : (slot ^ ((hx >> 1) & 3));
 }
 
-template <int TH, int WN, int PREC, bool RIDER, int NW = 8, bool RF = (NW == 4), bool GNB = false, bool DROP = false, bool GNC = false>
+template <int TH, int WN, int PREC, bool RIDER, int NW = 8, bool RF = (NW == 4), bool GNB = false, bool DROP = false, bool GNC = false, bool GS_ = false>
 __global__ void __launch_bounds__(64 * NW, 2) conv_k32_kernel(const ConvParams p) {
   using Cfg = ConvK32Cfg<TH, WN, PREC, NW>;
   constexpr int TW = Cfg::TW, KC = Cfg::KC, NP = Cfg::NP, ROWB = Cfg::ROWB, HWD = Cfg::HWD, NPIX = Cfg::NPIX;
@@ -210,9 +210,15 @@
     }
     __syncthreads();
   };
-  auto prefetch_rng = [&](int kc, QM* rin, auto i0_tag, auto i1_tag, bool load_gn) __attribute__((always_inline)) {
-    constexpr int I0 = decltype(i0_tag)::value, I1 = decltype(i1_tag)::value;
-    const ChunkSrc src = chunk_src<RIDER>(p, kc, KC, nk, q, gn);
+  typedef std::integral_constant<int, CHUNK_MAIN> K_MAIN;
+  typedef std::integral_constant<int, CHUNK_RIDER> K_RIDER;
+  typedef std::integral_constant<int, CHUNK_ANY> K_ANY;
+  typedef std::integral_constant<int, RIDER && !RFIRST ? CHUNK_ANY : CHUNK_MAIN> K_NEXT;
+  constexpr bool GS = GS_ || GNC || (DROP && NW == 4);
+  float satm = 0.f;
+  auto prefetch_rng = [&](int kc, QM* rin, auto i0_tag, auto i1_tag, bool load_gn, auto kind_tag) __attribute__((always_inline)) {
+    constexpr int I0 = decltype(i0_tag)::value, I1 = decltype(i1_tag)::value, KIND = decltype(kind_tag)::value;
+    const ChunkSrc src = chunk_src<RIDER, KIND>(p, kc, KC, nk, q, GS || gn);
     if (!GNC && src.gn && load_gn) {
       rsc = *reinterpret_cast<const f32x4*>(p.gn_scale + (size_t)n * Cin + src.cbase + q * 4);
       rsh = *reinterpret_cast<const f32x4*>(p.gn_shift + (size_t)n * Cin + src.cbase + q * 4);
@@ -222,14 +228,15 @@
       const size_t pi = (size_t)(in_pix[i] < 0 ? 0 : in_pix[i]);
       rin[i - I0].q = IO::load4(src.base, pi * src.Cs + src.cc);
       if (DROP)
-        rin[i - I0].m = *reinterpret_cast<const unsigned*>(p.drop_mask + ((RIDER && kc >= nk) ? (size_t)0 : pi * src.Cs + src.cc));
-    }
-  };
-  auto prefetch_to = [&](int kc, QM* rin) __attribute__((always_inline)) { prefetch_rng(kc, rin, I_0{}, I_N{}, true); };
-  auto stage_rng = [&](int kc, unsigned char* buf, const QM* rin, auto i0_tag, auto i1_tag) __attribute__((always_inline)) {
-    constexpr int I0 = decltype(i0_tag)::value, I1 = decltype(i1_tag)::value;
+        rin[i - I0].m = *reinterpret_cast<const unsigned*>(p.drop_mask + ((RIDER && chunk_is_rider<KIND>(kc, nk)) ? (size_t)0 : pi * src.Cs + src.cc));
+    }
+  };
+  auto prefetch_to = [&](int kc, QM* rin, auto kind_tag) __attribute__((always_inline)) { prefetch_rng(kc, rin, I_0{}, I_N{}, true, kind_tag); };
+  auto stage_rng = [&](int kc, unsigned char* buf, const QM* rin, auto i0_tag, auto i1_tag, auto kind_tag) __attribute__((always_inline)) {
+    constexpr int I0 = decltype(i0_tag)::value, I1 = decltype(i1_tag)::value, KIND = decltype(kind_tag)::value;
+    const bool rider = RIDER && chunk_is_rider<KIND>(kc, nk);
     f32x4 sc = rsc, sh = rsh;
-    if (GNC && !(RIDER && kc >= nk)) {
+    if (GNC && !rider) {
       sc = *reinterpret_cast<const f32x4*>(gnc_sc + (kc * KC - gnc_lo + q * 4));
       sh = *reinterpret_cast<const f32x4*>(gnc_sh + (kc * KC - gnc_lo + q * 4));
     }
@@ -240,16 +247,16 @@
       if (K32_DIAG & 16) v = sc;
       if ((K32_DIAG & 1) && gn) {
         v = v + sh;
-      } else if (gn && !(RIDER && kc >= nk)) {
+      } else if ((GS || gn) && !rider) {
         v = v * sc + sh;
-        if (!p.gn_plain) { v.x = silu_fast(v.x); v.y = silu_fast(v.y); v.z = silu_fast(v.z); v.w = silu_fast(v.w); }
+        if (GS || !p.gn_plain) { v.x = silu_fast(v.x); v.y = silu_fast(v.y); v.z = silu_fast(v.z); v.w = silu_fast(v.w); }
         if (DROP) {
           const unsigned m = rin[i - I0].m;
 #pragma unroll
           for (int e = 0; e < 4; ++e) v[e] *= (float)((m >> (8 * e)) & 0xffu) * p.drop_scale;
         }
-      } else if (PREC == PREC_F16X3 && p.sat_flag) {
-        sat_check(p.sat_flag, v, 65504.f);
+      } else if (PREC == PREC_F16X3) {
+        satm = sat_fold(satm, v);
       }
       const int sd = sbase + i * (RPP * ROWB) + 16 * ((q >> 1) ^ (int)((skeys >> (3 * i)) & 7u));
       unsigned char* dst = buf + sd;
@@ -275,16 +282,16 @@
       }
     }
   };
-  auto stage_from = [&](int kc, unsigned char* buf, const QM* rin) __attribute__((always_inline)) { stage_rng(kc, buf, rin, I_0{}, I_N{}); };
+  auto stage_from = [&](int kc, unsigned char* buf, const QM* rin, auto kind_tag) __attribute__((always_inline)) { stage_rng(kc, buf, rin, I_0{}, I_N{}, kind_tag); };
 
   const uint4* wq = reinterpret_cast<const uint4*>(p.wq);
   const int nkt = RIDER ? nk + nkr : nk;
   uint4 Wf[R][2][NP];
   const int wlane = 32 * (g & 1) + c15;
-  auto load_w = [&](int kc, int tap, int slot) __attribute__((always_inline)) {
+  auto load_w = [&](int kc, int tap, int slot, auto kind_tag) __attribute__((always_inline)) {
     if (K32_DIAG & 32) kc = 0;
     const uint4* src = wq + ((((size_t)cot * nk16 + 2 * kc + (g >> 1)) * WN + wn) * 9 + tap) * (Cfg::WNP * 64) + wlane;
-    if (RIDER && kc >= nk)
+    if (RIDER && chunk_is_rider<decltype(kind_tag)::value>(kc, nk))
       src = reinterpret_cast<const uint4*>(p.wq_r) + (((size_t)cot * p.nkr + 2 * (kc - nk) + (g >> 1)) * WN + wn) * (Cfg::WNP * 64) + wlane;
 #pragma unroll
     for (int ch = 0; ch < 2; ++ch)
@@ -309,35 +316,40 @@
       for (int ch = 0; ch < 2; ++ch) acc[mb][ph][ch] = f32x4{0.f, 0.f, 0.f, 0.f};
 
   const int kc0 = ksi * nkt / SK, kc1 = (ksi + 1) * nkt / SK;
-  if (RFIRST || (RIDER && kc0 >= nk)) load_w(RFIRST ? nk : kc0, 0, 0);
+  if (RFIRST) load_w(nk, 0, 0, K_RIDER{});
+  else if (RIDER && kc0 >= nk) load_w(kc0, 0, 0, K_RIDER{});
   else {
 #pragma unroll
-    for (int t = 0; t < R; ++t) load_w(kc0, t, t);
+    for (int t = 0; t < R; ++t) load_w(kc0, t, t, K_MAIN{});
   }
   const int gm0 = RFIRST ? 0 : (kc0 < nk ? kc0 : nk), gm1 = RIDER ? (kc1 < nk ? kc1 : nk) : kc1;
   const bool gnc_on = GNC && gm1 > gm0;
   if (gnc_on) gnc_issue(gm0 * KC, gm1 * KC < Cin ? gm1 * KC : Cin);
   if (RFIRST) {
+    if (!GNC && (GS || gn)) {
+      rsc = *reinterpret_cast<const f32x4*>(p.gn_scale + (size_t)n * Cin + q * 4);
+      rsh = *reinterpret_cast<const f32x4*>(p.gn_shift + (size_t)n * Cin + q * 4);
+    }
     {
       QM r0[NIN];
-      prefetch_to(nk, r0);
+      prefetch_to(nk, r0, K_RIDER{});
       if (gnc_on) gnc_finish();
-      stage_from(nk, sBuf0, r0);
-    }
-    prefetch_to(nkr > 1 ? nk + 1 : 0, rr1);
+      stage_from(nk, sBuf0, r0, K_RIDER{});
+    }
+    prefetch_rng(nkr > 1 ? nk + 1 : 0, rr1, I_0{}, I_N{}, false, K_ANY{});
   } else if (SPLIT) {
     {
       QM r0[NIN];
-      prefetch_to(kc0, r0);
+      prefetch_to(kc0, r0, K_NEXT{});
       if (gnc_on) gnc_finish();
-      stage_from(kc0, sBuf0, r0);
-    }
-    if (RIDER && kc0 >= nk && kc0 + 1 < kc1) prefetch_to(kc0 + 1, rr1);
+      stage_from(kc0, sBuf0, r0, K_NEXT{});
+    }
+    if (RIDER && kc0 >= nk && kc0 + 1 < kc1) prefetch_to(kc0 + 1, rr1, K_RIDER{});
   } else {
-    prefetch_to(kc0, rin);
+    prefetch_to(kc0, rin, K_NEXT{});
     if (gnc_on) gnc_finish();
-    stage_from(kc0, sBuf0, rin);
-    if (kc0 + 1 < kc1) prefetch_to(kc0 + 1, rin);
+    stage_from(kc0, sBuf0, rin, K_NEXT{});
+    if (kc0 + 1 < kc1) prefetch_to(kc0 + 1, rin, K_NEXT{});
   }
   __syncthreads();
 
@@ -397,7 +409,7 @@
     constexpr bool LAST = decltype(last_tag)::value;
     unsigned char* cur = ((kc - kc0 + par0) & 1) ? sBuf1 : sBuf0;
     unsigned char* nxt = ((kc - kc0 + par0) & 1) ? sBuf0 : sBuf1;
-    const bool more = LAST ? false : (kc + 1 < (RFIRST ? nk : kc1));
+    const bool more = LAST ? false : (RFIRST ? (PEEL ? true : kc + 1 < nk) : kc + 1 < kc1);
     const bool next_rider = RIDER && !RFIRST && kc + 1 >= nk;
 #pragma unroll
     for (int kx = 0; kx < 3; ++kx)
@@ -418,21 +430,21 @@
         mfma_step(s % XS, tap % R, mb);
         if (PIN) __builtin_amdgcn_sched_barrier(0);
       }
-      if (tap + R < 9) load_w(kc, tap + R, tap % R);
-      else if (more && (tap + R - 9 == 0 || !next_rider)) load_w(kc + 1, tap + R - 9, tap % R);
+      if (tap + R < 9) load_w(kc, tap + R, tap % R, K_MAIN{});
+      else if (more && (tap + R - 9 == 0 || !next_rider)) load_w(kc + 1, tap + R - 9, tap % R, K_NEXT{});
       if (SPLIT) {
-        if (tap == 0 && more) prefetch_rng(kc + 1, rin, I_0{}, I_A{}, true);
+        if (tap == 0 && more) prefetch_rng(kc + 1, rin, I_0{}, I_A{}, true, K_NEXT{});
         if (tap == 3 && more) {
-          if (!(K32_DIAG & 2)) stage_rng(kc + 1, nxt, rin, I_0{}, I_A{});
-          prefetch_rng(kc + 1, rin, I_A{}, I_N{}, false);
+          if (!(K32_DIAG & 2)) stage_rng(kc + 1, nxt, rin, I_0{}, I_A{}, K_NEXT{});
+          prefetch_rng(kc + 1, rin, I_A{}, I_N{}, false, K_NEXT{});
         }
         if (tap == 7 && more) {
-          if (!(K32_DIAG & 2)) stage_rng(kc + 1, nxt, rin, I_A{}, I_N{});
-          if (next_rider && kc + 2 < kc1) prefetch_to(kc + 2, rr1);
+          if (!(K32_DIAG & 2)) stage_rng(kc + 1, nxt, rin, I_A{}, I_N{}, K_NEXT{});
+          if (next_rider && kc + 2 < kc1) prefetch_to(kc + 2, rr1, K_RIDER{});
         }
       } else if (tap == 4 && more) {
-        stage_from(kc + 1, nxt, rin);
-        if (kc + 2 < kc1) prefetch_to(kc + 2, rin);
+        stage_from(kc + 1, nxt, rin, K_NEXT{});
+        if (kc + 2 < kc1) prefetch_to(kc + 2, rin, K_NEXT{});
       }
       if (LAST && res_early) {
         if (tap == 0) load_res(I_0{}, I_7{});
@@ -443,39 +455,40 @@
     }
     __syncthreads();
   };
+  auto rider_mfma = [&](unsigned char* cur) __attribute__((always_inline)) {
+#pragma unroll
+    for (int pl = 0; pl < NP; ++pl) xptr[1][pl] = cur + xoff[1][pl];
+#pragma unroll
+    for (int mb = 0; mb < XS - 1 && mb < MB; ++mb) load_x(mb, 1, 1, mb);
+#pragma unroll
+    for (int mb = 0; mb < MB; ++mb) {
+      if (mb + XS - 1 < MB) load_x((mb + XS - 1) % XS, 1, 1, mb + XS - 1);
+      mfma_step(mb % XS, 0, mb);
+    }
+  };
   if (RFIRST) {
-    for (int v = 0; v < nkr; ++v) {
-      unsigned char* cur = (v & 1) ? sBuf1 : sBuf0;
-      unsigned char* nxt = (v & 1) ? sBuf0 : sBuf1;
-#pragma unroll
-      for (int pl = 0; pl < NP; ++pl) xptr[1][pl] = cur + xoff[1][pl];
-#pragma unroll
-      for (int mb = 0; mb < XS - 1 && mb < MB; ++mb) load_x(mb, 1, 1, mb);
-#pragma unroll
-      for (int mb = 0; mb < MB; ++mb) {
-        if (mb + XS - 1 < MB) load_x((mb + XS - 1) % XS, 1, 1, mb + XS - 1);
-        mfma_step(mb % XS, 0, mb);
-      }
-      if (v + 1 < nkr) {
-        load_w(nk + v + 1, 0, 0);
-        stage_from(nk + v + 1, nxt, rr1);
-        prefetch_to(v + 2 < nkr ? nk + v + 2 : 0, rr1);
-      } else {
-#pragma unroll
-        for (int t = 0; t < R; ++t) load_w(0, t, t);
-        stage_from(0, nxt, rr1);
-      }
+    for (int v = 0; v + 1 < nkr; ++v) {
+      rider_mfma((v & 1) ? sBuf1 : sBuf0);
+      load_w(nk + v + 1, 0, 0, K_RIDER{});
+      stage_from(nk + v + 1, (v & 1) ? sBuf0 : sBuf1, rr1, K_RIDER{});
+      prefetch_rng(v + 2 < nkr ? nk + v + 2 : 0, rr1, I_0{}, I_N{}, false, K_ANY{});
       __syncthreads();
     }
-    {
-      const float ratio = (p.w_inv_scale_r_dev ? *p.w_inv_scale_r_dev : p.w_inv_scale_r) / (p.w_inv_scale_dev ? *p.w_inv_scale_dev : p.w_inv_scale);
-#pragma unroll
-      for (int mb = 0; mb < MB; ++mb)
-#pragma unroll
-        for (int ph = 0; ph < 2; ++ph)
-#pragma unroll
-          for (int ch = 0; ch < 2; ++ch) acc[mb][ph][ch] *= ratio;
-    }
+  }
+  if (RFIRST) {
+    const int v = nkr - 1;
+    rider_mfma((v & 1) ? sBuf1 : sBuf0);
+#pragma unroll
+    for (int t = 0; t < R; ++t) load_w(0, t, t, K_MAIN{});
+    stage_from(0, (v & 1) ? sBuf0 : sBuf1, rr1, K_MAIN{});
+    __syncthreads();
+    const float ratio = (p.w_inv_scale_r_dev ? *p.w_inv_scale_r_dev : p.w_inv_scale_r) / (p.w_inv_scale_dev ? *p.w_inv_scale_dev : p.w_inv_scale);
+#pragma unroll
+    for (int mb = 0; mb < MB; ++mb)
+#pragma unroll
+      for (int ph = 0; ph < 2; ++ph)
+#pragma unroll
+        for (int ch = 0; ch < 2; ++ch) acc[mb][ph][ch] *= ratio;
   }
   if (PEEL) {
     for (int kc = kc0; kc < kcm - 1; ++kc) main_chunk(kc, std::false_type{});
@@ -495,23 +508,14 @@
     }
     const int k0 = kc0 > nk ? kc0 : nk;
     constexpr int AH = K32_RIDER2 && NW == 8 ? 2 : 1;
-    if (AH == 2 && k0 + 2 < kc1) prefetch_to(k0 + 2, rin2);
+    if (AH == 2 && k0 + 2 < kc1) prefetch_to(k0 + 2, rin2, K_RIDER{});
     auto rider_chunk = [&](int kc, QM* r1) __attribute__((always_inline)) {
-      unsigned char* cur = ((kc - kc0) & 1) ? sBuf1 : sBuf0;
       unsigned char* nxt = ((kc - kc0) & 1) ? sBuf0 : sBuf1;
-#pragma unroll
-      for (int pl = 0; pl < NP; ++pl) xptr[1][pl] = cur + xoff[1][pl];
-#pragma unroll
-      for (int mb = 0; mb < XS - 1 && mb < MB; ++mb) load_x(mb, 1, 1, mb);
-#pragma unroll
-      for (int mb = 0; mb < MB; ++mb) {
-        if (mb + XS - 1 < MB) load_x((mb + XS - 1) % XS, 1, 1, mb + XS - 1);
-        mfma_step(mb % XS, 0, mb);
-      }
+      rider_mfma(((kc - kc0) & 1) ? sBuf1 : sBuf0);
       if (kc + 1 < kc1) {
-        load_w(kc + 1, 0, 0);
-        stage_from(kc + 1, nxt, r1);
-        if (kc + 1 + AH < kc1) prefetch_to(kc + 1 + AH, r1);
+        load_w(kc + 1, 0, 0, K_RIDER{});
+        stage_from(kc + 1, nxt, r1, K_RIDER{});
+        if (kc + 1 + AH < kc1) prefetch_to(kc + 1 + AH, r1, K_RIDER{});
       }
       __syncthreads();
     };
@@ -525,6 +529,8 @@
       for (int kc = k0; kc < kc1; ++kc) rider_chunk(kc, rfirst);
     }
   }
+
+  if (PREC == PREC_F16X3) sat_raise(p.sat_flag, satm, 65504.f);
 
   f32x4 add[2];
   bool cok[2];
@@ -784,6 +790,7 @@
   using IO = ActIO<PREC>;
   typedef typename IO::Quad Quad;
   Quad rin[NIN];
+  float satm = 0.f;
   auto prefetch = [&](int kc) {
     const size_t coff = (size_t)kc * KC + q * 4;
 #pragma unroll
@@ -796,7 +803,7 @@
       f32x4 v = IO::widen(rin[i]);
       const int sd = sbase + i * (RPP * ROWB) + 16 * ((q >> 1) ^ (int)((skeys >> (3 * i)) & 7u));
       if (PREC == PREC_F16X3) {
-        if (p.sat_flag) sat_check(p.sat_flag, v, 65504.f);
+        satm = sat_fold(satm, v);
         const float lim = in_pix[i] >= 0 ? 65504.f : 0.f;
 #pragma unroll
         for (int e = 0; e < 4; ++e) v[e] = __builtin_amdgcn_fmed3f(v[e], -lim, lim);
@@ -920,6 +927,7 @@
     }
     __syncthreads();
   }
+  if (PREC == PREC_F16X3) sat_raise(p.sat_flag, satm, 65504.f);
 
   const int cob = co0 + wn * 32 + 4 * g;
   const float winv = p.w_inv_scale_dev ? *p.w_inv_scale_dev : p.w_inv_scale;
@@ -1033,10 +1041,10 @@
   return true;
 }
 
-template <int TH, int WN, int PREC, bool RIDER, int NW = 8, bool RF = (NW == 4), bool GNB = false, bool DROP = false, bool GNC = false>
+template <int TH, int WN, int PREC, bool RIDER, int NW = 8, bool RF = (NW == 4), bool GNB = false, bool DROP = false, bool GNC = false, bool GS_ = false>
 static hipError_t launch_k32_t(const ConvParams& q, int nwg, hipStream_t s) {
   using Cfg = ConvK32Cfg<TH, WN, PREC, NW>;
-  hipLaunchKernelGGL((conv_k32_kernel<TH, WN, PREC, RIDER, NW, RF, GNB, DROP, GNC>), dim3(nwg), dim3(Cfg::NT), (size_t)Cfg::LDS_BYTES + (GNC ? K32_GNC_LDS : 0), s, q);
+  hipLaunchKernelGGL((conv_k32_kernel<TH, WN, PREC, RIDER, NW, RF, GNB, DROP, GNC, GS_>), dim3(nwg), dim3(Cfg::NT), (size_t)Cfg::LDS_BYTES + (GNC ? K32_GNC_LDS : 0), s, q);
   return hipGetLastError();
 }
 
@@ -1050,6 +1058,8 @@
   if (q.gb_G <= 0 || q.Cout % q.gb_G || q.Cout % 4) return false;
   return q.gb_x1 ? (q.gb_C0 % 4 == 0 && q.gb_C0 > 0 && q.gb_C0 < q.Cout) : q.gb_C0 == q.Cout;
 }
+
+static bool k32_gs(const ConvParams& q) { return q.gn_scale && !q.gn_plain; }
 
 static int k32_small_rows(int prec, bool rider) { return prec_is16(prec) && !rider ? 8 : 6; }
 
@@ -1076,8 +1086,10 @@
     if (!conv_k32_drop_ok(prec, q)) return hipErrorInvalidValue;
     return q.xr0 ? launch_k32_t<6, 2, PREC_F16X3, true, 4, true, false, true>(q, nwg, s) : launch_k32_t<6, 2, PREC_F16X3, false, 4, true, false, true>(q, nwg, s);
   }
-  if (prec == PREC_F16X3)
+  if (prec == PREC_F16X3) {
+    if (k32_gs(q)) return q.xr0 ? launch_k32_t<6, 2, PREC_F16X3, true, 4, true, false, false, false, true>(q, nwg, s) : launch_k32_t<6, 2, PREC_F16X3, false, 4, true, false, false, false, true>(q, nwg, s);
     return q.xr0 ? launch_k32_t<6, 2, PREC_F16X3, true, 4>(q, nwg, s) : launch_k32_t<6, 2, PREC_F16X3, false, 4>(q, nwg, s);
+  }
   if (prec == PREC_F16) return q.xr0 ? launch_k32_t<6, 2, PREC_F16, true, 4>(q, nwg, s) : launch_k32_t<8, 2, PREC_F16, false, 4>(q, nwg, s);
   return q.xr0 ? launch_k32_t<6, 2, PREC_BF16, true, 4>(q, nwg, s) : launch_k32_t<8, 2, PREC_BF16, false, 4>(q, nwg, s);
 }
@@ -1115,6 +1127,12 @@
       return q.xr0 ? launch_k32_t<TH_, WN_, PREC_F16X3, true, 8, true, false, true>(q, nwg, s)                  \
                    : launch_k32_t<TH_, WN_, PREC_F16X3, false, 8, false, false, true>(q, nwg, s);               \
     }                                                                                                           \
+    if (prec == PREC_F16X3 && k32_gs(q)) {                                                                      \
+      if (q.xr0 && q.ksplit <= 1 && (g_tun.k32 & FDSR_K32_RIDER_FIRST_8WAVE))                                   \
+        return launch_k32_t<TH_, WN_, PREC_F16X3, true, 8, true, false, false, false, true>(q, nwg, s);         \
+      return q.xr0 ? launch_k32_t<TH_, WN_, PREC_F16X3, true, 8, false, false, false, false, true>(q, nwg, s)   \
+                   : launch_k32_t<TH_, WN_, PREC_F16X3, false, 8, false, false, false, false, true>(q, nwg, s); \
+    }                                                                                                           \
     if (q.xr0 && q.ksplit <= 1 && (g_tun.k32 & FDSR_K32_RIDER_FIRST_8WAVE))                                                           \
       return prec == PREC_F16X3 ? launch_k32_t<TH_, WN_, PREC_F16X3, true, 8, true>(q, nwg, s)                  \
                                 : prec == PREC_F16 ? launch_k32_t<TH_, WN_, PREC_F16, true, 8, true>(q, nwg, s) : launch_k32_t<TH_, WN_, PREC_BF16, true, 8, true>(q, nwg, s);                  \
@@ -1128,9 +1146,9 @@
   return hipErrorInvalidValue;
 }
 
-template <int TH, int WN, int PREC, bool RIDER, int NW = 8, bool RF = (NW == 4), bool GNB = false, bool DROP = false, bool GNC = false>
+template <int TH, int WN, int PREC, bool RIDER, int NW = 8, bool RF = (NW == 4), bool GNB = false, bool DROP = false, bool GNC = false, bool GS_ = false>
 static hipError_t init_k32_t() {
-  auto kfn = conv_k32_kernel<TH, WN, PREC, RIDER, NW, RF, GNB, DROP, GNC>;
+  auto kfn = conv_k32_kernel<TH, WN, PREC, RIDER, NW, RF, GNB, DROP, GNC, GS_>;
   return hipFuncSetAttribute(reinterpret_cast<const void*>(kfn), hipFuncAttributeMaxDynamicSharedMemorySize, 160 * 1024);
 }
 
@@ -1156,6 +1174,9 @@
   if ((e = init_k32_t<TH_, WN_, PREC_BF16, true>()) != hipSuccess) return e;                \
   if ((e = init_k32_t<TH_, WN_, PREC_F16, true>()) != hipSuccess) return e;                \
   if ((e = init_k32_t<TH_, WN_, PREC_F16X3, true, 8, true>()) != hipSuccess) return e;     \
+  if ((e = init_k32_t<TH_, WN_, PREC_F16X3, false, 8, false, false, false, false, true>()) != hipSuccess) return e; \
+  if ((e = init_k32_t<TH_, WN_, PREC_F16X3, true, 8, false, false, false, false, true>()) != hipSuccess) return e;  \
+  if ((e = init_k32_t<TH_, WN_, PREC_F16X3, true, 8, true, false, false, false, true>()) != hipSuccess) return e;   \
   if ((e = init_k32_t<TH_, WN_, PREC_F16X3, false, 8, false, true>()) != hipSuccess) return e; \
   if ((e = init_k32_t<TH_, WN_, PREC_F16X3, false, 8, false, false, true>()) != hipSuccess) return e; \
   if ((e = init_k32_t<TH_, WN_, PREC_F16X3, true, 8, true, false, true>()) != hipSuccess) return e; \
@@ -1177,6 +1198,8 @@
 #undef X
   if ((e = init_k32_t<6, 2, PREC_F16X3, false, 4>()) != hipSuccess) return e;
   if ((e = init_k32_t<6, 2, PREC_F16X3, true, 4>()) != hipSuccess) return e;
+  if ((e = init_k32_t<6, 2, PREC_F16X3, false, 4, true, false, false, false, true>()) != hipSuccess) return e;
+  if ((e = init_k32_t<6, 2, PREC_F16X3, true, 4, true, false, false, false, true>()) != hipSuccess) return e;
   if ((e = init_k32_t<6, 2, PREC_F16X3, false, 4, true, true>()) != hipSuccess) return e;
   if ((e = init_k32_t<6, 2, PREC_F16X3, false, 4, true, false, true>()) != hipSuccess) return e;
   if ((e = init_k32_t<6, 2, PREC_F16X3, true, 4, true, false, true>()) != hipSuccess) return e;
diff --git a/fastdiffsr_amd/csrc/fdsr_conv_up2.hip b/fastdiffsr_amd/csrc/fdsr_conv_up2.hip
--- a/fastdiffsr_amd/csrc/fdsr_conv_up2.hip
+++ b/fastdiffsr_amd/csrc/fdsr_conv_up2.hip
@@ -54,6 +54,7 @@
   }
   using IO = ActIO<PREC>;
   typename IO::Quad rin[NIN];
+  float satm = 0.f;
   auto prefetch = [&](int kc) {
     const size_t coff = (size_t)kc * KC + q * 4;
 #pragma unroll
@@ -69,7 +70,7 @@
       const float lim = in_pix[i] >= 0 ? 65504.f : 0.f;
       unsigned char* dst = buf + (row0 + i * RPP) * ROWB + q * 8;
       if (PREC == PREC_F16X3) {
-        if (p.sat_flag) sat_check(p.sat_flag, v, 65504.f);
+        satm = sat_fold(satm, v);
         h4 hi, lo;
         split4_2step(v, lim, hi, lo);
         *reinterpret_cast<h4*>(dst) = hi;
@@ -146,6 +147,7 @@
     }
     __syncthreads();
   }
+  if (PREC == PREC_F16X3) sat_raise(p.sat_flag, satm, 65504.f);
 
   const int co = co0 + wn * 32 + r31;
   const bool cok = co < p.Cout;
```

Result: faster. 76.09 images/s, median of 6 (+1.9%).
